# alenzhao/Mitty

Measured on AMD Instinct MI355X. Metric: paired 2x150bp reads/sec at 30x WGS, 1/2/4/8 MI355X; qname POS/CIGAR bit-exact, higher is better.
Workload: dtype int64+u8

## Files before the change

### include/mitty_hip.h

```cpp
#ifndef MITTY_HIP_H
#define MITTY_HIP_H

#include <stdint.h>

#ifdef __cplusplus
extern "C" {
#endif

typedef struct mh_ctx mh_ctx;

enum {
  MH_OK = 0,
  MH_E_ARG = -1,
  MH_E_HIP = -2,
  MH_E_OOM = -3,
  MH_E_CAPACITY = -4,
  MH_E_COMPLEX_VARIANT = -5,
  MH_E_SEED = -6,
  MH_E_STATE = -7,
  MH_E_NO_DEVICE = -8
};

enum { MH_RNG_MITTY = 0, MH_RNG_PHILOX = 1 };

// ... 111 lines not shown
int32_t mh_bam_export(mh_ctx *ctx, int64_t r0, int64_t r1, uint8_t *recs, int64_t *roff, uint64_t *keys,
                      int32_t *info);
int32_t mh_bam_import(mh_ctx *ctx, const uint8_t *recs, const int64_t *roff, const uint64_t *keys, const int32_t *info,
                      int64_t n);
int32_t mh_bam_write_gpu(mh_ctx *ctx, const char *bam_path, const char *header_text, int64_t header_len,
                         const char *bai_path, int64_t *out_records, int64_t *out_bytes, int64_t *out_file_bytes);
int32_t mh_bam_partition(mh_ctx *ctx, const uint64_t *splitters, int32_t n_dest, uint64_t tie_base, int64_t *seg_off,
                         int64_t *seg_n, int64_t *seg_bytes);
int32_t mh_bam_partition_fetch(mh_ctx *ctx, void *out, int64_t cap);
int32_t mh_bam_import_tie(mh_ctx *ctx, const uint8_t *recs, const int64_t *roff, const uint64_t *keys,
                          const int32_t *info, const uint64_t *ties, int64_t n);
int32_t mh_bam_sorted_head(mh_ctx *ctx, int64_t len, uint8_t *out);
int32_t mh_bam_write_part(mh_ctx *ctx, const char *path, const char *header_text, int64_t header_len, int64_t skip,
                          const uint8_t *tail, int64_t tail_len, int32_t eof, int64_t *out_blocks, int64_t *out_data_pos,
                          int64_t *out_bytes, int64_t *boff, int64_t boff_cap);
int32_t mh_bam_bai_runs(mh_ctx *ctx, int64_t *n_runs, int64_t *runs, int64_t runs_cap, int64_t *n_win, int64_t *win,
                        int64_t win_cap, int64_t *ref_nwin);

typedef struct mh_bamfile mh_bamfile;
int32_t mh_bamfile_open(const char *path, int32_t threads, mh_bamfile **out);
const char *mh_bamfile_error(const mh_bamfile *f);
int32_t mh_bamfile_header(const mh_bamfile *f, const char **text, int64_t *text_len, int32_t *n_ref,
                          const char **names, const int64_t **lengths);
int32_t mh_bamfile_next(mh_bamfile *f, int64_t max_bytes, const uint8_t **recs, int64_t *len, const int64_t **roff,
                        int64_t *n);
int32_t mh_bamfile_close(mh_bamfile *f);

int32_t mh_score_begin(mh_ctx *ctx, int32_t n_refs, const char *names, int32_t max_d, int32_t max_v_len,
                       int32_t strict, const char *sample_prefix);
int32_t mh_score_add_records(mh_ctx *ctx, const uint8_t *recs, int64_t len, const int64_t *roff, int64_t n);
int32_t mh_score_add_store(mh_ctx *ctx);
int32_t mh_score_result(mh_ctx *ctx, uint64_t *mq_mat, uint64_t *derr_mat, int64_t *counts);
int32_t mh_score_reset(mh_ctx *ctx);

typedef struct mh_vcf mh_vcf;
int32_t mh_vcf_open(const char *path, const char *sample, mh_vcf **out);
const char *mh_vcf_error(const mh_vcf *v);
int32_t mh_vcf_close(mh_vcf *v);
int32_t mh_vcf_region(mh_vcf *v, const char *chrom, int64_t start0, int64_t end, int32_t *ploidy, int64_t *n_var,
                      int64_t *alt_bytes, int32_t cap);
int32_t mh_vcf_copy(mh_vcf *v, int32_t cpy, int64_t *pos, uint8_t *op, int64_t *oplen, int64_t *alt_off,
                    int64_t *alt_len, char *alt_pool);
int32_t mh_vcf_filter(const char *in_path, const char *sample, int32_t n_regions, const char *chroms,
                      const int64_t *start0, const int64_t *end, const char *out_path, int32_t bgzf, int32_t threads,
                      int64_t *n_written, int64_t *n_filtered, char *err, int32_t err_cap);

typedef struct mh_fasta mh_fasta;
int32_t mh_fasta_open(const char *path, const char *names, mh_fasta **out);
const char *mh_fasta_error(const mh_fasta *f);
int32_t mh_fasta_count(const mh_fasta *f, int32_t *n);
int32_t mh_fasta_contig(const mh_fasta *f, int32_t i, const char **name, const char **seq, int64_t *len);
int32_t mh_fasta_copy(const mh_fasta *f, int32_t i, char *dst);
int32_t mh_fasta_close(mh_fasta *f);

int32_t mh_bgzf_compress(const char *in, int64_t len, int32_t level, int32_t threads, char *out, int64_t cap,
                         int64_t *used);
int32_t mh_bgzf_eof(char *out28);
int32_t mh_bgzf_compress_device(mh_ctx *ctx, const void *d_in, int64_t len, void *d_out, int64_t cap,
                                int64_t *used);
int32_t mh_bgzf_compress_gpu(mh_ctx *ctx, const char *in, int64_t len, char *out, int64_t cap, int64_t *used);
int32_t mh_output_bgzf(mh_ctx *ctx, int32_t file, char *out, int64_t cap, int64_t *used);
int32_t mh_output_bgzf_range(mh_ctx *ctx, int32_t file, int64_t offset, int64_t len, char *out, int64_t cap,
                             int64_t *used);
int32_t mh_output_bgzf_pair(mh_ctx *ctx, int64_t offset, int64_t n1, int64_t n2, char *out1, int64_t cap1,
                            char *out2, int64_t cap2, int64_t *used1, int64_t *used2, int32_t *ticket);
int32_t mh_output_bgzf_wait(mh_ctx *ctx, int32_t ticket);

int32_t mh_corrupt_fastq(mh_ctx *ctx, const char *fq1, int64_t len1, const char *fq2, int64_t len2, int64_t t_base,
                         int64_t *used1, int64_t *used2, int64_t *templates);

int32_t mh_set_corruption(mh_ctx *ctx, int32_t enable, const double *cum_bq, int32_t max_bp, int32_t n_bq,
                          const double *phred_p, uint64_t seed);
int32_t mh_set_corruption_stream(mh_ctx *ctx, int32_t rng_mode, uint64_t seed, const uint32_t *key624, int32_t pos);
int32_t mh_get_corruption_stream(mh_ctx *ctx, uint32_t *key624, int32_t *pos, int64_t *words);

int32_t mh_stage_times(mh_ctx *ctx, const char **names, double *ms, int32_t cap, int32_t *n);
int32_t mh_enable_timing(mh_ctx *ctx, int32_t on);

int32_t mh_mt_window_at(uint32_t seed, uint64_t offset, uint32_t *out624);
int32_t mh_set_emit_mode(mh_ctx *ctx, int32_t mode);
#define MH_DEC_SEQUENTIAL 1
#define MH_DEC_FORCE_FIXUP 2
#define MH_DEC_FORCE_GEO 4
int32_t mh_set_decode_mode(mh_ctx *ctx, int32_t mode);
int32_t mh_fixup_count(mh_ctx *ctx, int64_t *n);

#ifdef __cplusplus
}
#endif
#endif
```

### mitty_amd/_native.py

```python
import ctypes
import os
import sys

import numpy as np

LIB_PATH = (os.environ.get('MH_LIB') or
            os.path.join(os.path.dirname(os.path.abspath(__file__)), '_lib', 'libmitty_hip.so'))

MH_OK, MH_E_ARG, MH_E_HIP, MH_E_OOM, MH_E_CAPACITY, MH_E_COMPLEX_VARIANT, MH_E_SEED, MH_E_STATE, MH_E_NO_DEVICE = \
  0, -1, -2, -3, -4, -5, -6, -7, -8
MH_RNG_MITTY, MH_RNG_PHILOX = 0, 1

EXPORTS = ['mh_version', 'mh_device_count', 'mh_create', 'mh_destroy', 'mh_last_error', 'mh_sync',
           'mh_selftest_scan_fault', 'mh_selftest_scan', 'mh_selftest_sort',
           'mh_read_model_params', 'mh_work_units', 'mh_upload_contig', 'mh_build_haplotype', 'mh_upload_variants', 'mh_build_haplotype_vset', 'mh_build_haplotypes_vset', 'mh_prefetch_haplotypes_vset', 'mh_release_variants', 'mh_get_nodes', 'mh_get_haplotype_aux',
           'mh_release_haplotype', 'mh_expand_variant', 'mh_sample_templates', 'mh_sample_templates_span', 'mh_set_templates',
           'mh_get_templates', 'mh_templates_export', 'mh_templates_import', 'mh_emit_reads', 'mh_emit_prepare', 'mh_emit_reads_async', 'mh_emit_collect', 'mh_output_size', 'mh_output_fetch', 'mh_output_reset', 'mh_host_alloc', 'mh_host_free', 'mh_device_cache_trim', 'mh_device_live_bytes',
           'mh_read_batch', 'mh_set_corruption', 'mh_set_corruption_stream', 'mh_get_corruption_stream', 'mh_stage_times', 'mh_enable_timing', 'mh_sample_units', 'mh_sample_units_async', 'mh_templates_count',
           'mh_use_templates', 'mh_release_templates', 'mh_mt_window_at', 'mh_fixup_count', 'mh_set_emit_mode', 'mh_set_decode_mode',
           'mh_emit_reads_range', 'mh_emit_measure', 'mh_count_kept', 'mh_bam_set_refs', 'mh_bam_add_fastq', 'mh_bam_add_output',
           'mh_bam_records', 'mh_bam_set_capacity', 'mh_bam_set_spill_dir', 'mh_bam_spilled', 'mh_bam_export', 'mh_bam_import', 'mh_bam_sort', 'mh_bam_write', 'mh_bam_write_gpu', 'mh_bam_reset', 'mh_bam_partition', 'mh_bam_partition_fetch', 'mh_bam_import_tie', 'mh_bam_sorted_head', 'mh_bam_write_part', 'mh_bam_bai_runs', 'mh_corrupt_fastq', 'mh_bgzf_compress', 'mh_bgzf_eof', 'mh_bgzf_compress_device', 'mh_bgzf_compress_gpu', 'mh_output_bgzf',
           'mh_output_bgzf_range', 'mh_output_bgzf_pair', 'mh_output_bgzf_wait', 'mh_output_fetch_async',
           'mh_output_fetch_wait',
           'mh_vcf_open', 'mh_vcf_error', 'mh_vcf_close', 'mh_vcf_region', 'mh_vcf_copy', 'mh_vcf_filter',
           'mh_bamfile_open', 'mh_bamfile_error', 'mh_bamfile_header', 'mh_bamfile_next', 'mh_bamfile_close',
           'mh_score_begin', 'mh_score_add_records', 'mh_score_add_store', 'mh_score_result', 'mh_score_reset',
           'mh_fasta_open', 'mh_fasta_error', 'mh_fasta_count', 'mh_fasta_contig', 'mh_fasta_copy', 'mh_fasta_close']


class NativeError(RuntimeError):
  pass


class NativeUnavailable(NativeError):
  pass


_lib = None

c_i32, c_i64, c_u64, c_dbl, c_vp = ctypes.c_int32, ctypes.c_int64, ctypes.c_uint64, ctypes.c_double, ctypes.c_void_p
P_i64 = ctypes.POINTER(c_i64)


def _sig(L, name, args, res=c_i32):
  f = getattr(L, name)
  f.argtypes = args
  f.restype = res


def lib():
  global _lib
  if _lib is not None:
    return _lib
  if not os.path.exists(LIB_PATH):
    raise NativeUnavailable('libmitty_hip.so not built ({}); run __graft_entry__.build() or make -C '
                            'mitty_amd/csrc'.format(LIB_PATH))
  if 'torch' not in sys.modules and int(os.environ.get('WORLD_SIZE', '1')) > 1:
    import torch
  L = ctypes.CDLL(LIB_PATH)
  _sig(L, 'mh_version', [])
  _sig(L, 'mh_device_count', [ctypes.POINTER(c_i32)])
  _sig(L, 'mh_create', [c_i32, ctypes.POINTER(c_vp)])
  _sig(L, 'mh_destroy', [c_vp])
  _sig(L, 'mh_last_error', [c_vp], ctypes.c_char_p)
  _sig(L, 'mh_sync', [c_vp])
  _sig(L, 'mh_selftest_scan_fault', [c_vp])
  _sig(L, 'mh_selftest_scan', [c_vp, c_i32, c_i32, c_vp, c_i64, c_i32, c_vp, c_vp, c_vp, c_vp])
  _sig(L, 'mh_selftest_sort', [c_vp, c_vp, c_i64, c_i32, c_vp, c_vp])
  _sig(L, 'mh_read_model_params', [c_i64, c_dbl, ctypes.POINTER(c_dbl), P_i64])
  _sig(L, 'mh_work_units', [c_u64, c_vp, c_i64, c_i64, c_vp, c_vp, c_vp, P_i64])
  _sig(L, 'mh_upload_contig', [c_vp, c_i32, c_vp, c_i64])
  _sig(L, 'mh_upload_variants', [c_vp, c_i32, c_vp, c_vp, c_vp, c_vp, c_vp, c_vp, c_i64, c_i64])
  _sig(L, 'mh_build_haplotype_vset', [c_vp, c_i32, c_i32, c_i64, c_i32, c_vp, c_vp, c_vp])
  _sig(L, 'mh_release_variants', [c_vp, c_i32])
  _sig(L, 'mh_build_haplotype', [c_vp, c_i32, c_i32, c_i64, c_vp, c_vp, c_vp, c_vp, c_vp, c_vp, c_i64, c_i64,
                                 P_i64, P_i64, P_i64])
  _sig(L, 'mh_get_nodes', [c_vp, c_i32, c_vp, c_vp, c_vp, c_vp, c_vp, c_i64, P_i64])
  _sig(L, 'mh_get_haplotype_aux', [c_vp, c_i32, c_vp, c_i64, P_i64, c_vp, c_vp, c_i64, P_i64, c_vp, c_i64, P_i64])
  _sig(L, 'mh_release_haplotype', [c_vp, c_i32])
  _sig(L, 'mh_bgzf_compress_device', [c_vp, c_vp, c_i64, c_vp, c_i64, P_i64])
  _sig(L, 'mh_bgzf_compress_gpu', [c_vp, c_vp, c_i64, c_vp, c_i64, P_i64])
  _sig(L, 'mh_output_bgzf', [c_vp, c_i32, c_vp, c_i64, P_i64])
  _sig(L, 'mh_output_bgzf_range', [c_vp, c_i32, c_i64, c_i64, c_vp, c_i64, P_i64])
  _sig(L, 'mh_output_bgzf_pair', [c_vp, c_i64, c_i64, c_i64, c_vp, c_i64, c_vp, c_i64, P_i64, P_i64,
                                  ctypes.POINTER(c_i32)])
  _sig(L, 'mh_output_bgzf_wait', [c_vp, c_i32])
  _sig(L, 'mh_output_fetch_async', [c_vp, c_i64, c_vp, c_i64, c_i64, c_vp, c_i64, ctypes.POINTER(c_i32)])
  _sig(L, 'mh_output_fetch_wait', [c_vp, c_i32])
  _sig(L, 'mh_expand_variant', [c_i64, c_i64, c_i64, c_i64, c_i32, c_i64, P_i64, ctypes.POINTER(c_i32), P_i64, P_i64])
  _sig(L, 'mh_sample_templates', [c_vp, c_i32, c_dbl, c_i32, c_vp, c_i32, c_u64, c_i32, P_i64])
  _sig(L, 'mh_sample_templates_span', [c_vp, c_i64, c_i64, c_dbl, c_i32, c_vp, c_i32, c_u64, c_i32, P_i64])
  _sig(L, 'mh_set_templates', [c_vp, c_vp, c_vp, c_vp, c_i64, c_i32])
  _sig(L, 'mh_get_templates', [c_vp, c_vp, c_vp, c_vp, c_i64, P_i64])
  _sig(L, 'mh_emit_reads', [c_vp, c_i32, ctypes.c_char_p, ctypes.c_char_p, c_i64, c_i32, c_u64, P_i64, P_i64, P_i64])
  _sig(L, 'mh_emit_prepare', [c_vp, c_i32, ctypes.c_char_p, ctypes.c_char_p, c_i64, c_i32, c_u64, P_i64, P_i64, P_i64])
  _sig(L, 'mh_emit_reads_async', [c_vp, c_i32, ctypes.c_char_p, ctypes.c_char_p, c_i64, c_i32, c_u64])
  _sig(L, 'mh_emit_collect', [c_vp, c_vp, c_i64, P_i64])
  _sig(L, 'mh_build_haplotypes_vset', [c_vp, c_i32, c_vp, c_vp, c_vp, c_vp, c_vp, c_vp, c_vp])
  _sig(L, 'mh_prefetch_haplotypes_vset', [c_vp, c_i32, c_vp, c_vp, c_vp, c_vp, c_i32, c_vp, c_vp, c_dbl])
  _sig(L, 'mh_emit_reads_range', [c_vp, c_i32, ctypes.c_char_p, ctypes.c_char_p, c_i64, c_i32, c_u64, c_i64, c_i64,
                                   c_i64, P_i64, P_i64, P_i64])
  _sig(L, 'mh_count_kept', [c_vp, c_i32, c_i64, c_i64, P_i64])
  _sig(L, 'mh_emit_measure', [c_vp, c_i32, ctypes.c_char_p, ctypes.c_char_p, c_i64, c_i32, c_u64, c_i64, c_i64, c_i64,
                              P_i64, P_i64, P_i64])
  _sig(L, 'mh_bam_set_refs', [c_vp, c_i32, ctypes.c_char_p, c_vp])
  _sig(L, 'mh_bam_add_fastq', [c_vp, c_vp, c_i64, c_vp, c_i64, c_i64, P_i64, P_i64, P_i64])
  _sig(L, 'mh_bam_add_output', [c_vp, c_i64, P_i64])
  _sig(L, 'mh_bam_records', [c_vp, P_i64, P_i64])
  _sig(L, 'mh_bam_set_capacity', [c_vp, c_i64])
  _sig(L, 'mh_bam_spilled', [c_vp, P_i64, P_i64])
  _sig(L, 'mh_bam_export', [c_vp, c_i64, c_i64, c_vp, c_vp, c_vp, c_vp])
  _sig(L, 'mh_bam_import', [c_vp, c_vp, c_vp, c_vp, c_vp, c_i64])
  _sig(L, 'mh_bam_partition', [c_vp, c_vp, c_i32, ctypes.c_uint64, c_vp, c_vp, c_vp])
  _sig(L, 'mh_bam_set_spill_dir', [c_vp, ctypes.c_char_p])
  _sig(L, 'mh_bam_partition_fetch', [c_vp, c_vp, c_i64])
  _sig(L, 'mh_bam_import_tie', [c_vp, c_vp, c_vp, c_vp, c_vp, c_vp, c_i64])
  _sig(L, 'mh_bam_sorted_head', [c_vp, c_i64, c_vp])
  _sig(L, 'mh_bam_write_part', [c_vp, ctypes.c_char_p, ctypes.c_char_p, c_i64, c_i64, c_vp, c_i64, c_i32, P_i64,
                                P_i64, P_i64, c_vp, c_i64])
  _sig(L, 'mh_bam_bai_runs', [c_vp, P_i64, c_vp, c_i64, P_i64, c_vp, c_i64, c_vp])
  _sig(L, 'mh_bam_write', [c_vp, ctypes.c_char_p, ctypes.c_char_p, c_i64, c_i32, c_i32, ctypes.c_char_p, P_i64,
                           P_i64])
  _sig(L, 'mh_bam_write_gpu', [c_vp, ctypes.c_char_p, ctypes.c_char_p, c_i64, ctypes.c_char_p, P_i64, P_i64, P_i64])
  _sig(L, 'mh_bam_reset', [c_vp])
  _sig(L, 'mh_bam_sort', [c_vp])
  _sig(L, 'mh_corrupt_fastq', [c_vp, c_vp, c_i64, c_vp, c_i64, c_i64, P_i64, P_i64, P_i64])
  _sig(L, 'mh_bgzf_compress', [c_vp, c_i64, c_i32, c_i32, c_vp, c_i64, P_i64])
  _sig(L, 'mh_bgzf_eof', [c_vp])
  _sig(L, 'mh_vcf_open', [ctypes.c_char_p, ctypes.c_char_p, ctypes.POINTER(c_vp)])
  _sig(L, 'mh_vcf_error', [c_vp], ctypes.c_char_p)
  _sig(L, 'mh_vcf_close', [c_vp])
  _sig(L, 'mh_vcf_region', [c_vp, ctypes.c_char_p, c_i64, c_i64, ctypes.POINTER(c_i32), c_vp, c_vp, c_i32])
  _sig(L, 'mh_vcf_copy', [c_vp, c_i32, c_vp, c_vp, c_vp, c_vp, c_vp, c_vp])
  _sig(L, 'mh_vcf_filter', [ctypes.c_char_p, ctypes.c_char_p, c_i32, c_vp, c_vp, c_vp, ctypes.c_char_p, c_i32, c_i32,
                            P_i64, P_i64, ctypes.c_char_p, c_i32])
  _sig(L, 'mh_bamfile_open', [ctypes.c_char_p, c_i32, ctypes.POINTER(c_vp)])
  _sig(L, 'mh_bamfile_error', [c_vp], ctypes.c_char_p)
  _sig(L, 'mh_bamfile_header', [c_vp, ctypes.POINTER(c_vp), P_i64, ctypes.POINTER(c_i32), ctypes.POINTER(c_vp),
                                ctypes.POINTER(c_vp)])
  _sig(L, 'mh_bamfile_next', [c_vp, c_i64, ctypes.POINTER(c_vp), P_i64, ctypes.POINTER(c_vp), P_i64])
  _sig(L, 'mh_bamfile_close', [c_vp])
  _sig(L, 'mh_score_begin', [c_vp, c_i32, ctypes.c_char_p, c_i32, c_i32, c_i32, ctypes.c_char_p])
  _sig(L, 'mh_score_add_records', [c_vp, c_vp, c_i64, c_vp, c_i64])
  _sig(L, 'mh_score_add_store', [c_vp])
  _sig(L, 'mh_score_result', [c_vp, c_vp, c_vp, c_vp])
  _sig(L, 'mh_score_reset', [c_vp])
  _sig(L, 'mh_fasta_open', [ctypes.c_char_p, c_vp, ctypes.POINTER(c_vp)])
  _sig(L, 'mh_fasta_error', [c_vp], ctypes.c_char_p)
  _sig(L, 'mh_fasta_count', [c_vp, ctypes.POINTER(c_i32)])
  _sig(L, 'mh_fasta_contig', [c_vp, c_i32, ctypes.POINTER(ctypes.c_char_p), ctypes.POINTER(c_vp), P_i64])
  _sig(L, 'mh_fasta_copy', [c_vp, c_i32, c_vp])
  _sig(L, 'mh_fasta_close', [c_vp])
  _sig(L, 'mh_output_size', [c_vp, P_i64, P_i64])
  _sig(L, 'mh_output_fetch', [c_vp, c_i64, c_vp, c_i64, c_i64, c_vp, c_i64])
  _sig(L, 'mh_output_reset', [c_vp])
  _sig(L, 'mh_host_alloc', [c_i64, ctypes.POINTER(c_vp)])
  _sig(L, 'mh_host_free', [c_vp])
  _sig(L, 'mh_device_cache_trim', [ctypes.POINTER(c_i64)])
  _sig(L, 'mh_device_live_bytes', [ctypes.POINTER(c_i64), ctypes.POINTER(c_i64), c_i32])
  _sig(L, 'mh_read_batch', [c_vp, c_i32, c_vp, c_vp, c_i64, c_vp, c_vp, c_vp,
                            c_vp, c_i64, c_vp, P_i64, c_vp, c_i64, c_vp, P_i64, c_vp, c_i64, c_vp, P_i64])
  _sig(L, 'mh_set_corruption', [c_vp, c_i32, c_vp, c_i32, c_i32, c_vp, c_u64])
  _sig(L, 'mh_templates_export', [c_vp, c_i32, c_i32, c_vp, c_vp, c_vp, c_i64, P_i64])
  _sig(L, 'mh_templates_import', [c_vp, c_i32, c_i32, c_vp, c_vp, c_vp, c_i64, c_i32])
  _sig(L, 'mh_set_corruption_stream', [c_vp, c_i32, c_u64, c_vp, c_i32])
  _sig(L, 'mh_get_corruption_stream', [c_vp, c_vp, ctypes.POINTER(c_i32), P_i64])
  _sig(L, 'mh_stage_times', [c_vp, ctypes.POINTER(ctypes.c_char_p), ctypes.POINTER(c_dbl), c_i32,
                             ctypes.POINTER(c_i32)])
  _sig(L, 'mh_enable_timing', [c_vp, c_i32])
  _sig(L, 'mh_sample_units', [c_vp, c_i32, c_vp, c_vp, c_vp, c_dbl, c_i32, c_vp, c_i32, c_i32, c_vp])
  _sig(L, 'mh_sample_units_async', [c_vp, c_i32, c_vp, c_vp, c_vp, c_dbl, c_i32, c_vp, c_i32, c_i32])
  _sig(L, 'mh_templates_count', [c_vp, c_i32, c_vp])
  _sig(L, 'mh_use_templates', [c_vp, c_i32])
  _sig(L, 'mh_release_templates', [c_vp, c_i32])
  _sig(L, 'mh_mt_window_at', [ctypes.c_uint32, c_u64, c_vp])
  _sig(L, 'mh_fixup_count', [c_vp, P_i64])
  _sig(L, 'mh_set_emit_mode', [c_vp, c_i32])
  _sig(L, 'mh_set_decode_mode', [c_vp, c_i32])
  _lib = L
  return L


def mt_window_at(seed, offset):
  out = np.empty(624, np.uint32)
  rc = lib().mh_mt_window_at(int(seed), int(offset), _ptr(out))
  if rc:
    _raise(rc, 'mh_mt_window_at failed')
  return out


def bgzf_compress(data, level=6, threads=8):
  n = len(data)
  src = np.frombuffer(data, np.uint8) if n else np.zeros(1, np.uint8)
  cap = n + (n // 0xff00 + 1) * 64 + 64
  out = np.empty(cap, np.uint8)
  used = c_i64()
  rc = lib().mh_bgzf_compress(_ptr(src), n, int(level), int(threads), _ptr(out), cap, ctypes.byref(used))
  if rc == MH_E_CAPACITY:
    out = np.empty(used.value, np.uint8)
    rc = lib().mh_bgzf_compress(_ptr(src), n, int(level), int(threads), _ptr(out), used.value, ctypes.byref(used))
  if rc:
    _raise(rc, 'mh_bgzf_compress failed')
  return out[:used.value].tobytes()


class VcfFile:

  def __init__(self, path, sample):
    L = lib()
    self._L = L
    self._h = c_vp()
    rc = L.mh_vcf_open(path.encode(), sample.encode(), ctypes.byref(self._h))
    if rc:
      msg = L.mh_vcf_error(self._h).decode() if self._h else 'mh_vcf_open failed'
      self.close()
      _raise(rc, msg)

  def close(self):
    if getattr(self, '_h', None):
      self._L.mh_vcf_close(self._h)
      self._h = None

  def __del__(self):
    try:
      self.close()
    except Exception:
      pass

  def region(self, chrom, start0, end):
    pl = c_i32()
    nv = np.zeros(64, np.int64)
    ab = np.zeros(64, np.int64)
    rc = self._L.mh_vcf_region(self._h, chrom.encode(), int(start0), int(end), ctypes.byref(pl), _ptr(nv), _ptr(ab),
                               64)
    if rc:
      _raise(rc, self._L.mh_vcf_error(self._h).decode())
    copies = []
    for c in range(pl.value):
      n, nb = int(nv[c]), int(ab[c])
      pos, oplen, aoff, alen = (np.empty(n, np.int64) for _ in range(4))
      op = np.empty(n, np.uint8)
      pool = np.empty(max(nb, 1), np.uint8)
      rc = self._L.mh_vcf_copy(self._h, c, _ptr(pos), _ptr(op), _ptr(oplen), _ptr(aoff), _ptr(alen), _ptr(pool))
      if rc:
        _raise(rc, self._L.mh_vcf_error(self._h).decode())
      copies.append({'pos': pos, 'op': op, 'oplen': oplen, 'alt_off': aoff, 'alt_len': alen,
                     'alt_pool': pool[:nb].tobytes()})
    return pl.value, copies


class BamFile:

  def __init__(self, path, threads=2):
    L = lib()
    self._L = L
    self._h = c_vp()
    rc = L.mh_bamfile_open(path.encode(), int(threads), ctypes.byref(self._h))
    if rc:
      msg = L.mh_bamfile_error(self._h).decode(errors='replace') if self._h else 'mh_bamfile_open failed'
# ... 269 lines not shown
    self._chk(self._L.mh_release_variants(self._h, int(vset)))

  def get_nodes(self, slot, n_nodes, with_hap=True):
    ps, pr, ol = (np.empty(max(n_nodes, 1), np.int64) for _ in range(3))
    op = np.empty(max(n_nodes, 1), np.uint8)
    hl = c_i64()
    self._chk(self._L.mh_get_nodes(self._h, slot, None, None, None, None, None, 0, ctypes.byref(hl)))
    hap = np.empty(max(hl.value, 1), np.uint8) if with_hap else None
    self._chk(self._L.mh_get_nodes(self._h, slot, _ptr(ps), _ptr(pr), _ptr(op), _ptr(ol), _ptr(hap),
                                   hl.value if with_hap else 0, ctypes.byref(hl)))
    return ps[:n_nodes], pr[:n_nodes], op[:n_nodes], ol[:n_nodes], (hap[:hl.value].tobytes() if with_hap else None)

  def get_haplotype_aux(self, slot):
    hl, nr, nb = c_i64(), c_i64(), c_i64()
    self._chk(self._L.mh_get_haplotype_aux(self._h, slot, None, 0, ctypes.byref(hl), None, None, 0, ctypes.byref(nr),
                                           None, 0, ctypes.byref(nb)))
    rc = np.empty(max(hl.value, 1), np.uint8)
    rs, re_ = np.empty(max(nr.value, 1), np.int64), np.empty(max(nr.value, 1), np.int64)
    bkt = np.empty(nb.value + 1, np.int32)
    self._chk(self._L.mh_get_haplotype_aux(self._h, slot, _ptr(rc), hl.value, ctypes.byref(hl), _ptr(rs), _ptr(re_),
                                           nr.value, ctypes.byref(nr), _ptr(bkt), nb.value + 1, ctypes.byref(nb)))
    return rc[:hl.value].tobytes(), rs[:nr.value], re_[:nr.value], bkt

  def release_haplotype(self, slot):
    self._chk(self._L.mh_release_haplotype(self._h, slot))

  def sample_templates(self, slot, p, rlen, cum_tlen, seed, rng_mode=MH_RNG_MITTY):
    ct = np.ascontiguousarray(cum_tlen, dtype=np.float64)
    n = c_i64()
    self._chk(self._L.mh_sample_templates(self._h, slot, float(p), int(rlen), _ptr(ct), len(ct), int(seed),
                                          int(rng_mode), ctypes.byref(n)))
    return n.value

  def sample_templates_span(self, p_min, p_max, p, rlen, cum_tlen, seed, rng_mode=MH_RNG_MITTY):
    if not (0 <= int(seed) <= 0xffffffff):
      raise ValueError('Seed value {} is out of range 0 - {}'.format(seed, 0xffffffff))
    ct = np.ascontiguousarray(cum_tlen, dtype=np.float64)
    n = c_i64()
    self._chk(self._L.mh_sample_templates_span(self._h, int(p_min), int(p_max), float(p), int(rlen), _ptr(ct),
                                               len(ct), int(seed), int(rng_mode), ctypes.byref(n)))
    return n.value

  def sample_units(self, tpl_ids, slots, seeds, p, rlen, cum_tlen, rng_mode=MH_RNG_MITTY):
    ids = np.ascontiguousarray(tpl_ids, dtype=np.int32)
    sl = np.ascontiguousarray(slots, dtype=np.int32)
    sd = np.ascontiguousarray(seeds, dtype=np.uint64)
    ct = np.ascontiguousarray(cum_tlen, dtype=np.float64)
    out = np.zeros(max(len(ids), 1), dtype=np.int64)
    self._chk(self._L.mh_sample_units(self._h, len(ids), _ptr(ids), _ptr(sl), _ptr(sd), float(p), int(rlen),
                                      _ptr(ct), len(ct), int(rng_mode), _ptr(out)))
    return out[:len(ids)]

  def sample_units_async(self, tpl_ids, slots, seeds, p, rlen, cum_tlen, rng_mode=MH_RNG_MITTY):
    ids = np.ascontiguousarray(tpl_ids, dtype=np.int32)
    sl = np.ascontiguousarray(slots, dtype=np.int32)
    sd = np.ascontiguousarray(seeds, dtype=np.uint64)
    ct = np.ascontiguousarray(cum_tlen, dtype=np.float64)
    self._chk(self._L.mh_sample_units_async(self._h, len(ids), _ptr(ids), _ptr(sl), _ptr(sd), float(p), int(rlen),
                                            _ptr(ct), len(ct), int(rng_mode)))
    return len(ids)

  def template_count(self, tpl_id):
    n = c_i64()
    self._chk(self._L.mh_templates_count(self._h, int(tpl_id), ctypes.byref(n)))
    return n.value

  def use_templates(self, tpl_id):
    self._chk(self._L.mh_use_templates(self._h, int(tpl_id)))

  def release_templates(self, tpl_id):
    self._chk(self._L.mh_release_templates(self._h, int(tpl_id)))

  def set_emit_mode(self, mode):
    self._chk(self._L.mh_set_emit_mode(self._h, int(mode)))

  def set_decode_mode(self, mode):
    self._chk(self._L.mh_set_decode_mode(self._h, int(mode)))

  def fixup_count(self):
    n = c_i64()
    self._chk(self._L.mh_fixup_count(self._h, ctypes.byref(n)))
    return n.value

  def set_templates(self, fo0, pos0, pos1, rlen):
    fo0 = np.ascontiguousarray(fo0, dtype=np.int8)
    pos0 = np.ascontiguousarray(pos0, dtype=np.int64)
    pos1 = np.ascontiguousarray(pos1, dtype=np.int64)
    self._chk(self._L.mh_set_templates(self._h, _ptr(fo0), _ptr(pos0), _ptr(pos1), len(fo0), int(rlen)))

  def get_templates(self):
    n = c_i64()
    self._L.mh_get_templates(self._h, None, None, None, 0, ctypes.byref(n))
    m = n.value
    fo0, p0, p1 = np.empty(max(m, 1), np.int8), np.empty(max(m, 1), np.int64), np.empty(max(m, 1), np.int64)
    self._chk(self._L.mh_get_templates(self._h, _ptr(fo0), _ptr(p0), _ptr(p1), max(m, 1), ctypes.byref(n)))
    return fo0[:m], p0[:m], p1[:m]

  def emit_prepare(self, slot, serial_stub, chrom, cpy, write_fastq2=True, unit_key=0, wait=True):
    if not wait:
      self._chk(self._L.mh_emit_prepare(self._h, slot, serial_stub.encode(), chrom.encode(), int(cpy),
                                        1 if write_fastq2 else 0, int(unit_key), None, None, None))
      return None
    k, b1, b2 = c_i64(), c_i64(), c_i64()
    self._chk(self._L.mh_emit_prepare(self._h, slot, serial_stub.encode(), chrom.encode(), int(cpy),
                                      1 if write_fastq2 else 0, int(unit_key), ctypes.byref(k), ctypes.byref(b1),
                                      ctypes.byref(b2)))
    return k.value, b1.value, b2.value

  def emit_reads(self, slot, serial_stub, chrom, cpy, write_fastq2=True, unit_key=0, t_range=None, cnt_base=0):
    k, b1, b2 = c_i64(), c_i64(), c_i64()
    if t_range is None:
      self._chk(self._L.mh_emit_reads(self._h, slot, serial_stub.encode(), chrom.encode(), int(cpy),
                                      1 if write_fastq2 else 0, int(unit_key), ctypes.byref(k), ctypes.byref(b1),
                                      ctypes.byref(b2)))
    else:
      self._chk(self._L.mh_emit_reads_range(self._h, slot, serial_stub.encode(), chrom.encode(), int(cpy),
                                            1 if write_fastq2 else 0, int(unit_key), int(t_range[0]),
                                            int(t_range[1]), int(cnt_base), ctypes.byref(k), ctypes.byref(b1),
                                            ctypes.byref(b2)))
    return k.value, b1.value, b2.value

  def emit_async(self, slot, serial_stub, chrom, cpy, write_fastq2=True, unit_key=0):
    self._chk(self._L.mh_emit_reads_async(self._h, slot, serial_stub.encode(), chrom.encode(), int(cpy),
                                          1 if write_fastq2 else 0, int(unit_key)))

  def emit_collect(self):
    n = c_i64()
    self._chk(self._L.mh_emit_collect(self._h, None, 0, ctypes.byref(n)))
    out = np.zeros(3 * max(n.value, 1), np.int64)
    self._chk(self._L.mh_emit_collect(self._h, _ptr(out), n.value, ctypes.byref(n)))
    return [tuple(int(x) for x in out[3 * i:3 * i + 3]) for i in range(n.value)]

  def emit_measure(self, slot, serial_stub, chrom, cpy, write_fastq2=True, unit_key=0, t_range=None, cnt_base=0):
    k, b1, b2 = c_i64(), c_i64(), c_i64()
    t0, t1 = t_range if t_range is not None else (0, -1)
    self._chk(self._L.mh_emit_measure(self._h, slot, serial_stub.encode(), chrom.encode(), int(cpy),
                                      1 if write_fastq2 else 0, int(unit_key), int(t0), int(t1), int(cnt_base),
                                      ctypes.byref(k), ctypes.byref(b1), ctypes.byref(b2)))
    return k.value, b1.value, (b2.value if write_fastq2 else 0)

  def bgzf_range(self, f, off, n, pin):
    if n <= 0:
      return b''
    cap = n + (n // 0xff00 + 2) * 40 + 64
    pin.reserve(cap)
    used = c_i64()
    self._chk(self._L.mh_output_bgzf_range(self._h, int(f), int(off), int(n), c_vp(pin.ptr), cap, ctypes.byref(used)))
    return bytes(pin.view(used.value))

  def count_kept(self, slot, t_begin, t_end):
    k = c_i64()
    self._chk(self._L.mh_count_kept(self._h, slot, int(t_begin), int(t_end), ctypes.byref(k)))
    return k.value

  def output_size(self):
    a, b = c_i64(), c_i64()
    self._chk(self._L.mh_output_size(self._h, ctypes.byref(a), ctypes.byref(b)))
    return a.value, b.value

  def fetch_output(self, off1=0, len1=None, off2=0, len2=None):
    u1, u2 = self.output_size()
    len1 = u1 - off1 if len1 is None else len1
    len2 = u2 - off2 if len2 is None else len2
    b1 = np.empty(max(len1, 1), np.uint8)
    b2 = np.empty(max(len2, 1), np.uint8)
    self._chk(self._L.mh_output_fetch(self._h, off1, _ptr(b1), len1, off2, _ptr(b2) if len2 > 0 else None, len2))
# ... 368 lines not shown
```

### mitty_amd/csrc/mh_api.hip

```cpp
#include <sys/mman.h>
#include <sys/syscall.h>
#include <unistd.h>

#include <algorithm>
#include <atomic>
#include <cctype>
#include <cstdio>
#include <unordered_map>
#include <chrono>
#include <cmath>
#include <condition_variable>
#include <cstring>
#include <map>
#include <mutex>
#include <thread>
#include <type_traits>

#include "mh_bgzf.h"
#include <vector>

#include "mh_corrupt.h"
#include "mh_internal.h"
#include "mh_scan.h"
#include "mh_sort.h"

namespace mh {
namespace jump {
void window_at(uint32_t seed, uint64_t J, uint32_t *out624);
}

static std::mutex g_err_mu;

int32_t hip_fail(mh_ctx *ctx, hipError_t e, const char *what, const char *file, int line) {
  if (ctx) {
    std::lock_guard<std::mutex> lk(g_err_mu);
    ctx->err = std::string("HIP error ") + hipGetErrorName(e) + " (" + hipGetErrorString(e) + ") in " + what + " at " +
               file + ":" + std::to_string(line);
  }
  return e == hipErrorOutOfMemory ? MH_E_OOM : MH_E_HIP;
}

int32_t arg_fail(mh_ctx *ctx, int32_t code, const std::string &msg) {
  if (ctx) {
    std::lock_guard<std::mutex> lk(g_err_mu);
    ctx->err = msg;
  }
  return code;
}

bool scan_fault_pending(const mh_ctx *ctx) {
  const uint32_t *h = scan_fault_host();
  return h && __atomic_load_n(h + (ctx ? ctx->fault_slot : 0), __ATOMIC_ACQUIRE) != 0;
}

void lane_thread_enter(mh_ctx *ctx) { scan_fault_slot = ctx->fault_slot; }

int32_t scan_fault_fail(mh_ctx *ctx) {
  const uint32_t v = scan_fault_take(ctx ? ctx->fault_slot : 0);
  if (v & 2u) return arg_fail(ctx, MH_E_STATE, "single-pass writer: a qname part exceeded the splice's bound (internal)");
  if (v & 4u) return arg_fail(ctx, MH_E_STATE, "single-pass writer: the arena reservation was too small (internal)");
  return arg_fail(ctx, MH_E_STATE, "a look-back scan's wait timed out (a broken ticket base or scratch): its offsets "
                                   "are wrong");
}

namespace {
struct CachedBlock {
  void *p;
  int dev;
};
std::mutex g_cache_mu;
std::multimap<size_t, CachedBlock> g_cache;
std::atomic<int64_t> g_live{0}, g_live_peak{0};

void live_add(int64_t d) {
  const int64_t v = g_live.fetch_add(d) + d;
  int64_t pk = g_live_peak.load();
  while (v > pk && !g_live_peak.compare_exchange_weak(pk, v)) {
  }
}

void cache_put(void *p, size_t cap) {
  live_add(-(int64_t)cap);
  int dev = 0;
  (void)hipGetDevice(&dev);
  (void)hipDeviceSynchronize();
  std::lock_guard<std::mutex> lk(g_cache_mu);
  g_cache.insert({cap, CachedBlock{p, dev}});
}

void *cache_take(size_t bytes, size_t *cap) {
  int dev = 0;
  (void)hipGetDevice(&dev);
  std::lock_guard<std::mutex> lk(g_cache_mu);
  for (auto it = g_cache.lower_bound(bytes); it != g_cache.end(); ++it)
    if (it->second.dev == dev) {
      void *p = it->second.p;
      *cap = it->first;
      g_cache.erase(it);
      return p;
    }
  return nullptr;
}

int64_t cache_trim(int dev) {
  std::vector<std::pair<void *, int>> out;
  int64_t freed = 0;
  {
    std::lock_guard<std::mutex> lk(g_cache_mu);
    for (auto it = g_cache.begin(); it != g_cache.end();)
      if (dev < 0 || it->second.dev == dev) {
        out.push_back({it->second.p, it->second.dev});
        freed += (int64_t)it->first;
        it = g_cache.erase(it);
      } else {
        ++it;
      }
  }
  int cur = 0;
  (void)hipGetDevice(&cur);
  for (auto &b : out) {
    if (b.second != cur) (void)hipSetDevice(b.second);
    (void)hipFree(b.first);
    if (b.second != cur) (void)hipSetDevice(cur);
  }
  return freed;
}

hipError_t dev_alloc(void **p, size_t bytes, size_t *cap) {
  if ((*p = cache_take(bytes, cap))) {
    live_add((int64_t)*cap);
    return hipSuccess;
  }
  hipError_t e = hipMalloc(p, bytes);
  if (e != hipSuccess) {
    (void)hipGetLastError();
    int dev = 0;
    (void)hipGetDevice(&dev);
    if (cache_trim(dev) > 0) e = hipMalloc(p, bytes);
  }
  if (e == hipSuccess) {
    *cap = bytes;
// ... 211 lines not shown
  __device__ void operator()(int64_t i, const T &in, const T &ex) const {
    incl[i] = in;
    excl[i] = ex;
  }
};

template <typename T>
int32_t selftest_scan_run(mh_ctx *ctx, int32_t kind, const int64_t *in, int64_t n, int32_t repeat, int64_t *incl,
                          int64_t *excl, int64_t *total, int64_t *info) {
  hipStream_t st = ctx->stream;
  MH_TRY(ensure(ctx, ctx->scan_partials,
                kind == 2 ? scan_lb_scratch_bytes<T>(n) : sizeof(T) * (size_t)scan_partials_count(n) + 64));
  DevBuf b;
  const size_t ab = (sizeof(T) * (size_t)n + 255) & ~(size_t)255;
  MH_TRY(ensure(ctx, b, 3 * ab + 256));
  T *d_in = (T *)b.p, *d_incl = (T *)((char *)b.p + ab), *d_excl = (T *)((char *)b.p + 2 * ab);
  T *d_tot = (T *)((char *)b.p + 3 * ab);
  const int32_t rc = [&]() -> int32_t {
    if (n) HIPCHK(ctx, hipMemcpyAsync(d_in, in, sizeof(T) * (size_t)n, hipMemcpyHostToDevice, st));
    HIPCHK(ctx, hipMemsetAsync(d_incl, 0xff, 2 * ab + 256, st));
    const LoadArr<T> load{d_in};
    const StoreBoth<T> store{d_incl, d_excl};
    for (int32_t r = 0; r < repeat; r++) {
      if (kind == 0)
        HIPCHK(ctx, device_scan<T>(st, n, load, store, OpSum{}, T{}, (T *)ctx->scan_partials.p, d_tot));
      else if (kind == 1) {
        if constexpr (std::is_same<T, int64_t>::value)
          HIPCHK(ctx, device_scan<T>(st, n, load, store, OpMax{}, INT64_MIN, (T *)ctx->scan_partials.p, d_tot));
      } else if (kind == 2)
        HIPCHK(ctx, device_scan_sum<T>(st, n, load, store, ctx->scan_partials.p, d_tot));
      else
        HIPCHK(ctx, device_reduce<T>(st, n, load, OpSum{}, T{}, (T *)ctx->scan_partials.p, d_tot));
    }
    if (kind == 2) {
      std::lock_guard<std::mutex> lk(lb_mu());
      auto it = lb_states().find(ctx->scan_partials.p);
      if (it == lb_states().end()) return arg_fail(ctx, MH_E_HIP, "the look-back scratch has no state after a launch");
      info[0] = (int64_t)it->second.epoch;
      info[1] = (int64_t)(it->second.ticket - (uint32_t)scan_partials_count(n));
    }
    if (n && kind != 3) {
      HIPCHK(ctx, hipMemcpyAsync(incl, d_incl, sizeof(T) * (size_t)n, hipMemcpyDeviceToHost, st));
      HIPCHK(ctx, hipMemcpyAsync(excl, d_excl, sizeof(T) * (size_t)n, hipMemcpyDeviceToHost, st));
    }
    HIPCHK(ctx, hipMemcpyAsync(total, d_tot, sizeof(T), hipMemcpyDeviceToHost, st));
    SYNCCHK(ctx, hipStreamSynchronize(st));
    return MH_OK;
  }();
  release(b);
  return rc;
}
static_assert(LB_TILE == SCAN_TILE, "selftest_scan_run counts look-back tiles with scan_partials_count");
}

extern "C" {

int32_t mh_version(void) { return 1; }

int32_t mh_device_count(int32_t *out) {
  int n = 0;
  hipError_t e = hipGetDeviceCount(&n);
  if (e != hipSuccess) {
    (void)hipGetLastError();
    n = 0;
  }
  *out = n;
  return MH_OK;
}

int32_t mh_create(int32_t device, mh_ctx **out) {
  if (!out) return MH_E_ARG;
  *out = nullptr;
  int n = 0;
  if (hipGetDeviceCount(&n) != hipSuccess || n == 0) {
    (void)hipGetLastError();
    return MH_E_NO_DEVICE;
  }
  if (device < 0 || device >= n) return MH_E_ARG;
  mh_ctx *ctx = new mh_ctx();
  ctx->device = device;
  {
    static std::atomic<int> next{0};
    ctx->fault_slot = 1 + next++ % (SCAN_FAULT_SLOTS - 1);
    (void)scan_fault_take(ctx->fault_slot);
  }
  int prio_lo = 0, prio_hi = 0;
  (void)hipSetDevice(device);
  (void)hipDeviceGetStreamPriorityRange(&prio_lo, &prio_hi);
  if (hipSetDevice(device) != hipSuccess ||
      hipStreamCreateWithPriority(&ctx->stream, hipStreamNonBlocking, prio_hi) != hipSuccess ||
      hipStreamCreateWithPriority(&ctx->stream2, hipStreamNonBlocking, prio_hi) != hipSuccess ||
      hipEventCreateWithFlags(&ctx->ev_fork, hipEventDisableTiming) != hipSuccess ||
      hipEventCreateWithFlags(&ctx->ev_join, hipEventDisableTiming) != hipSuccess ||
      hipStreamCreateWithPriority(&ctx->wstream, hipStreamNonBlocking, prio_lo) != hipSuccess ||
      hipEventCreateWithFlags(&ctx->ev_ready, hipEventDisableTiming) != hipSuccess ||
      hipEventCreateWithFlags(&ctx->ev_writer, hipEventDisableTiming) != hipSuccess ||
      [&] {
        for (auto &e : ctx->eset)
          if (hipEventCreateWithFlags(&e.done, hipEventDisableTiming) != hipSuccess ||
              hipEventCreateWithFlags(&e.rb, hipEventDisableTiming) != hipSuccess ||
              hipHostMalloc((void **)&e.h_stat, 64 + 8192, hipHostMallocDefault) != hipSuccess)
            return true;
        return false;
      }()) {
    delete ctx;
    return MH_E_HIP;
  }
  hipDeviceProp_t prop;
  if (hipGetDeviceProperties(&prop, device) == hipSuccess) ctx->max_cu = prop.multiProcessorCount;
  *out = ctx;
  return MH_OK;
}

int32_t mh_destroy(mh_ctx *ctx) {
  if (!ctx) return MH_OK;
  if (ctx->pf_thread.joinable()) ctx->pf_thread.join();
  (void)hipSetDevice(ctx->device);
  (void)hipStreamSynchronize(ctx->wstream);
  (void)hipStreamSynchronize(ctx->stream);
  if (ctx->stream2) (void)hipStreamSynchronize(ctx->stream2);
  if (ctx->pstream) (void)hipStreamSynchronize(ctx->pstream);
  for (auto x : ctx->xstream)
    if (x) (void)hipStreamSynchronize(x);
  for (auto &kv : ctx->contigs) release(kv.second.seq);
  for (auto &kv : ctx->haps) release_hap(kv.second);
  for (auto &h : ctx->hap_spare) release_hap(h);
  for (auto &kv : ctx->vsets) release_vars(kv.second);
  for (auto &kv : ctx->tsets) {
    release(kv.second.fo0); release(kv.second.pos0); release(kv.second.pos1); release(kv.second.n0);
    if (kv.second.used) (void)hipEventDestroy(kv.second.used);
  }
  release(ctx->jump_polys); release(ctx->perm_tmp); release(ctx->nrun_tmp); release(ctx->dec_buf);
  for (auto &b : ctx->pb) release(b);
  release(ctx->pb_tmp);
  release(ctx->gz_slots); release(ctx->gz_tok); release(ctx->gz_info); release(ctx->gz_off); release(ctx->gz_scan); release(ctx->gz_out);
  release(ctx->gz_in);
  for (auto &b : ctx->s) release(b);
  for (auto &b : ctx->lane2) release(b);
  for (auto &l : ctx->xlane)
    for (auto &b : l) release(b);
  for (auto &b : ctx->xscan) release(b);
  release(ctx->scan_partials); release(ctx->scan_partials2); release(ctx->d_small);
  release(ctx->corrupt_cum); release(ctx->corrupt_phred);
  release(ctx->out1); release(ctx->out2);
  release(ctx->cr_rows);
  release(ctx->cr_codes);
  release(ctx->scan_partials_w);
  for (auto &b : ctx->sl2) release(b);
  for (auto &b : ctx->sl3) release(b);
  ctx->tail_state.reset();
  for (hipEvent_t e : ctx->ev_gz)
    if (e) (void)hipEventDestroy(e);
  for (hipEvent_t e : ctx->ev_fetch)
    if (e) (void)hipEventDestroy(e);
  if (ctx->h_small) (void)hipHostFree(ctx->h_small);
  if (ctx->h_small3) (void)hipHostFree(ctx->h_small3);
  if (ctx->h_units) (void)hipHostFree(ctx->h_units);
  for (uint8_t *p : ctx->h_bam_pin)
    if (p) (void)hipHostFree(p);
  for (auto &e : ctx->eset) {
    release(e.recs); release(e.off); release(e.tsum); release(e.tpre); release(e.stat); release(e.crrec);
    (void)hipEventDestroy(e.done);
    if (e.rb) (void)hipEventDestroy(e.rb);
    if (e.h_stat) (void)hipHostFree(e.h_stat);
  }
  (void)hipEventDestroy(ctx->ev_ready);
  (void)hipEventDestroy(ctx->ev_writer);
// ... 20 lines not shown
  CTX_GUARD(ctx);
  MH_TRY(lazy_resolve(ctx));
  SYNCCHK(ctx, hipStreamSynchronize(ctx->stream));
  return MH_OK;
}

namespace {
struct LoadOne {
  __device__ int64_t operator()(int64_t) const { return 1; }
};
struct StoreCheck {
  int32_t *bad;
  __device__ void operator()(int64_t i, int64_t, int64_t ex) const {
    if (ex != i) atomicOr(bad, 1);
  }
};
}

int32_t mh_selftest_sort(mh_ctx *ctx, const uint32_t *keys, int64_t n, int32_t end_bit, uint32_t *keys_out,
                         uint32_t *vals_out) {
  CTX_GUARD(ctx);
  if (n < 0 || (n > 0 && (!keys || !keys_out || !vals_out)) || end_bit < 0 || end_bit > 32)
    return arg_fail(ctx, MH_E_ARG, "bad sort arguments");
  hipStream_t st = ctx->stream;
  size_t tmp = 0;
  HIPCHK(ctx, lsd_sort_pairs_iota(nullptr, tmp, nullptr, nullptr, nullptr, n, (unsigned)end_bit, st));
  DevBuf b;
  const size_t kb = (4 * (size_t)n + 255) & ~(size_t)255;
  MH_TRY(ensure(ctx, b, 3 * kb + tmp + 256));
  uint32_t *dk = (uint32_t *)b.p, *ko = (uint32_t *)((char *)b.p + kb), *vo = (uint32_t *)((char *)b.p + 2 * kb);
  const int32_t rc = [&]() -> int32_t {
    if (n) HIPCHK(ctx, hipMemcpyAsync(dk, keys, 4 * (size_t)n, hipMemcpyHostToDevice, st));
    HIPCHK(ctx, lsd_sort_pairs_iota((char *)b.p + 3 * kb, tmp, dk, ko, vo, n, (unsigned)end_bit, st));
    if (n) {
      HIPCHK(ctx, hipMemcpyAsync(keys_out, ko, 4 * (size_t)n, hipMemcpyDeviceToHost, st));
      HIPCHK(ctx, hipMemcpyAsync(vals_out, vo, 4 * (size_t)n, hipMemcpyDeviceToHost, st));
    }
    SYNCCHK(ctx, hipStreamSynchronize(st));
    return MH_OK;
  }();
  release(b);
  return rc;
}

int32_t mh_selftest_scan(mh_ctx *ctx, int32_t kind, int32_t fields, const int64_t *in, int64_t n, int32_t repeat,
                         int64_t *incl, int64_t *excl, int64_t *total, int64_t *info) {
  CTX_GUARD(ctx);
  if (kind < 0 || kind > 3 || fields < 1 || fields > 3 || (kind == 1 && fields != 1) || n < 0 ||
      n > ((int64_t)1 << 27) || repeat < 1 || repeat > (1 << 20) || ((kind == 1 || kind == 3) && repeat != 1) ||
      !total || !info || (n > 0 && (!in || (kind != 3 && (!incl || !excl)))))
    return arg_fail(ctx, MH_E_ARG, "bad scan self-test arguments");
  if (kind == 2) {
    uint64_t sum[3] = {0, 0, 0};
    for (int64_t i = 0; i < n * fields; i++) {
      if (in[i] < 0) return arg_fail(ctx, MH_E_ARG, "look-back scan: a negative input");
      uint64_t &s = sum[i % fields];
      s += (uint64_t)in[i];
      if (s >= ((uint64_t)1 << 46)) return arg_fail(ctx, MH_E_ARG, "look-back scan: a field's total is 2^46 or more");
    }
  }
  info[0] = info[1] = 0;
  if (fields == 1) return selftest_scan_run<int64_t>(ctx, kind, in, n, repeat, incl, excl, total, info);
  if (fields == 2) return selftest_scan_run<Sc2>(ctx, kind, in, n, repeat, incl, excl, total, info);
  return selftest_scan_run<Sc3>(ctx, kind, in, n, repeat, incl, excl, total, info);
}

int32_t mh_selftest_scan_fault(mh_ctx *ctx) {
  CTX_GUARD(ctx);
  hipStream_t st = ctx->stream;
  const int64_t n = 2 * (int64_t)LB_TILE + 5;
  MH_TRY(ensure(ctx, ctx->scan_partials, scan_lb_scratch_bytes<int64_t>(n)));
  MH_TRY(ensure(ctx, ctx->scan_partials2, scan_lb_scratch_bytes<int64_t>(n)));
  MH_TRY(ensure(ctx, ctx->d_small, 8192 + 256));
  int64_t *tot = (int64_t *)((char *)ctx->d_small.p + 160);
  int32_t *bad = (int32_t *)((char *)ctx->d_small.p + 168);
  auto fault_once = [&](hipStream_t s, void *scratch) -> int32_t {
    HIPCHK(ctx, hipMemsetAsync(bad, 0, 4, s));
    HIPCHK(ctx, device_scan_sum<int64_t>(s, n, LoadOne{}, StoreCheck{bad}, scratch, tot, true));
    SYNCCHK(ctx, hipStreamSynchronize(s));
    return MH_OK;
  };
  int32_t rc_lane = MH_OK;
  std::thread t1([&]() {
    lane_thread_enter(ctx);
    if (hipSetDevice(ctx->device) != hipSuccess) {
      rc_lane = MH_E_HIP;
      return;
    }
    rc_lane = fault_once(ctx->stream2, ctx->scan_partials2.p);
  });
  t1.join();
  if (rc_lane != MH_E_STATE) return arg_fail(ctx, MH_E_HIP, "the timed-out scan of a lane thread was not reported");
  const int32_t rc = fault_once(st, ctx->scan_partials.p);
  if (rc != MH_E_STATE) return arg_fail(ctx, MH_E_HIP, "the timed-out scan was not reported");
  const std::string msg = ctx->err;
  HIPCHK(ctx, hipMemsetAsync(bad, 0, 4, st));
  HIPCHK(ctx, device_scan_sum<int64_t>(st, n, LoadOne{}, StoreCheck{bad}, ctx->scan_partials.p, tot));
  int32_t hb = 0;
  HIPCHK(ctx, hipMemcpyAsync(&hb, bad, 4, hipMemcpyDeviceToHost, st));
  SYNCCHK(ctx, hipStreamSynchronize(st));
  if (hb) return arg_fail(ctx, MH_E_HIP, "the scan after the fault is wrong");
  arg_fail(ctx, MH_E_STATE, msg);
  return MH_E_STATE;
}

int32_t mh_read_model_params(int64_t mean_rlen, double coverage, double *p_out, int64_t *passes_out) {
  if (!p_out || !passes_out || mean_rlen <= 0) return MH_E_ARG;
  double p = 1.0;
  int64_t passes = 1;
  while (p > 0.1) {
    passes *= 2;
    p = 0.5 * coverage / (double)(2 * mean_rlen * passes);
  }
  *p_out = p;
  *passes_out = passes;
  return MH_OK;
}

int32_t mh_work_units(uint64_t seed, const int32_t *ploidy, int64_t n_regions, int64_t passes, int32_t *out_region,
                      int32_t *out_cpy, uint32_t *out_seed, int64_t *out_n) {
  if (seed > 0xffffffffull) return MH_E_SEED;
  if (n_regions < 0 || passes < 0 || (n_regions && !ploidy)) return MH_E_ARG;
  HostMT s;
  s.seed((uint32_t)seed);
  uint32_t shuffle_seed = (uint32_t)s.interval(0xfffffffeull);
  int64_t n = 0;
  for (int64_t r = 0; r < n_regions; r++)
    for (int32_t c = 0; c < ploidy[r]; c++)
      for (int64_t k = 0; k < passes; k++) {
        out_region[n] = (int32_t)r;
        out_cpy[n] = c;
        out_seed[n] = (uint32_t)s.interval(0xfffffffeull);
        n++;
      }
  HostMT sh;
  sh.seed(shuffle_seed);
  for (int64_t i = n - 1; i >= 1; i--) {
    int64_t j = (int64_t)sh.interval((uint64_t)i);
    std::swap(out_region[i], out_region[j]);
    std::swap(out_cpy[i], out_cpy[j]);
    std::swap(out_seed[i], out_seed[j]);
  }
  *out_n = n;
  return MH_OK;
}

int32_t mh_upload_contig(mh_ctx *ctx, int32_t contig_id, const char *seq, int64_t len) {
  CTX_GUARD(ctx);
  if (len < 0 || (len > 0 && !seq)) return arg_fail(ctx, MH_E_ARG, "bad contig");
  Contig &c = ctx->contigs[contig_id];
  MH_TRY(ensure(ctx, c.seq, len + 16));
  if (len) HIPCHK(ctx, hipMemcpyAsync(c.seq.p, seq, len, hipMemcpyHostToDevice, ctx->stream));
  SYNCCHK(ctx, hipStreamSynchronize(ctx->stream));
  c.len = len;
  return MH_OK;
}

static int32_t hap_for_build(mh_ctx *ctx, int32_t slot, int64_t need, Hap **out, hipStream_t st = nullptr) {
  if (!ctx->haps.count(slot)) {
    int best = -1, big = -1;
    for (int i = 0; i < (int)ctx->hap_spare.size(); i++) {
      const Hap &s = ctx->hap_spare[i];
      if (s.used_set && hipEventQuery(s.used) != hipSuccess) continue;
      if (s.hap.cap >= (size_t)need && (best < 0 || s.hap.cap < ctx->hap_spare[best].hap.cap)) best = i;
      if (big < 0 || s.hap.cap > ctx->hap_spare[big].hap.cap) big = i;
    }
    if (best < 0) best = big;
// ... 13 lines not shown
  *out = &h;
  return MH_OK;
}

static int32_t build_from(mh_ctx *ctx, int32_t slot, int32_t contig_id, int64_t ref_start_pos, const VarSet &v,
                          int64_t *out_n_nodes, int64_t *out_p_min, int64_t *out_p_max) {
  auto it = ctx->contigs.find(contig_id);
  if (it == ctx->contigs.end()) return arg_fail(ctx, MH_E_STATE, "unknown contig id");
  Hap *hp = nullptr;
  MH_TRY(hap_for_build(ctx, slot, it->second.len + (it->second.len >> 6) + (1 << 20), &hp));
  Hap &h = *hp;
  MH_TRY(splice_build(ctx, h, it->second, ref_start_pos, v));
  if (out_n_nodes) *out_n_nodes = h.n_nodes;
  if (out_p_min) *out_p_min = h.p_min;
  if (out_p_max) *out_p_max = h.p_max;
  return MH_OK;
}

int32_t mh_build_haplotype(mh_ctx *ctx, int32_t slot, int32_t contig_id, int64_t ref_start_pos, const int64_t *v_pos,
                           const uint8_t *v_op, const int64_t *v_oplen, const int64_t *v_alt_off,
                           const int64_t *v_alt_len, const char *alt_pool, int64_t alt_pool_len, int64_t n_var,
                           int64_t *out_n_nodes, int64_t *out_p_min, int64_t *out_p_max) {
  CTX_GUARD_NOJOIN(ctx);
  if (!ctx->contigs.count(contig_id)) return arg_fail(ctx, MH_E_STATE, "unknown contig id");
  if (n_var < 0 || (n_var > 0 && (!v_pos || !v_op || !v_oplen || !v_alt_off || !v_alt_len)))
    return arg_fail(ctx, MH_E_ARG, "bad variant arrays");
  VarSet &v = ctx->vsets[-1];
  MH_TRY(var_upload(ctx, v, v_pos, v_op, v_oplen, v_alt_off, v_alt_len, alt_pool, alt_pool_len, n_var));
  return build_from(ctx, slot, contig_id, ref_start_pos, v, out_n_nodes, out_p_min, out_p_max);
}

int32_t mh_upload_variants(mh_ctx *ctx, int32_t vset, const int64_t *v_pos, const uint8_t *v_op,
                           const int64_t *v_oplen, const int64_t *v_alt_off, const int64_t *v_alt_len,
                           const char *alt_pool, int64_t alt_pool_len, int64_t n_var) {
  CTX_GUARD(ctx);
  if (vset < 0) return arg_fail(ctx, MH_E_ARG, "variant set ids are >= 0");
  if (n_var < 0 || (n_var > 0 && (!v_pos || !v_op || !v_oplen || !v_alt_off || !v_alt_len)))
    return arg_fail(ctx, MH_E_ARG, "bad variant arrays");
  const int32_t rc = var_upload(ctx, ctx->vsets[vset], v_pos, v_op, v_oplen, v_alt_off, v_alt_len, alt_pool,
                                alt_pool_len, n_var);
  if (rc != MH_OK) {
    release_vars(ctx->vsets[vset]);
    ctx->vsets.erase(vset);
  }
  return rc;
}

int32_t mh_build_haplotype_vset(mh_ctx *ctx, int32_t slot, int32_t contig_id, int64_t ref_start_pos, int32_t vset,
                                int64_t *out_n_nodes, int64_t *out_p_min, int64_t *out_p_max) {
  CTX_GUARD_NOJOIN(ctx);
  auto it = ctx->vsets.find(vset);
  if (vset < 0 || it == ctx->vsets.end()) return arg_fail(ctx, MH_E_STATE, "unknown variant set id");
  return build_from(ctx, slot, contig_id, ref_start_pos, it->second, out_n_nodes, out_p_min, out_p_max);
}

int32_t mh_build_haplotypes_vset(mh_ctx *ctx, int32_t n, const int32_t *slots, const int32_t *contig_ids,
                                 const int64_t *ref_starts, const int32_t *vsets, int64_t *out_n_nodes,
                                 int64_t *out_p_min, int64_t *out_p_max) {
  CTX_GUARD_NOJOIN(ctx);
  if (n < 0 || (n > 0 && (!slots || !contig_ids || !ref_starts || !vsets))) return arg_fail(ctx, MH_E_ARG, "bad arguments");
  for (int32_t i = 0; i < n; i++) {
    if (!ctx->contigs.count(contig_ids[i])) return arg_fail(ctx, MH_E_STATE, "unknown contig id");
    if (vsets[i] < 0 || !ctx->vsets.count(vsets[i])) return arg_fail(ctx, MH_E_STATE, "unknown variant set id");
    for (int32_t j = 0; j < i; j++)
      if (slots[j] == slots[i]) return arg_fail(ctx, MH_E_ARG, "a slot appears twice");
  }
  if (!pinned_small(ctx)) return arg_fail(ctx, MH_E_OOM, "pinned host memory");
  for (int32_t i0 = 0; i0 < n; i0 += 2) {
    const int32_t k = n - i0 < 2 ? n - i0 : 2;
    Hap *hp[2] = {nullptr, nullptr};
    for (int32_t j = 0; j < k; j++) {
      const int64_t L = ctx->contigs[contig_ids[i0 + j]].len;
      MH_TRY(hap_for_build(ctx, slots[i0 + j], L + (L >> 6) + (1 << 20), &hp[j]));
    }
    if (k == 1) {
      MH_TRY(splice_build(ctx, *hp[0], ctx->contigs[contig_ids[i0]], ref_starts[i0], ctx->vsets[vsets[i0]]));
    } else {
      HIPCHK(ctx, hipEventRecord(ctx->ev_fork, ctx->stream));
      HIPCHK(ctx, hipStreamWaitEvent(ctx->stream2, ctx->ev_fork, 0));
      const Contig &c1 = ctx->contigs[contig_ids[i0 + 1]];
      const VarSet &v1 = ctx->vsets[vsets[i0 + 1]];
      int32_t rc1 = MH_OK;
      std::thread t1([&]() {
        lane_thread_enter(ctx);
        try {
          const hipError_t e = hipSetDevice(ctx->device);
          if (e != hipSuccess) {
            rc1 = hip_fail(ctx, e, "hipSetDevice (splice lane 1)", __FILE__, __LINE__);
            return;
          }
          rc1 = splice_build(ctx, *hp[1], c1, ref_starts[i0 + 1], v1, 1);
        } catch (const std::bad_alloc &) {
          rc1 = arg_fail(ctx, MH_E_OOM, "host memory (splice lane 1)");
        } catch (const std::exception &x) {
          rc1 = arg_fail(ctx, MH_E_STATE, std::string("splice lane 1: ") + x.what());
        } catch (...) {
          rc1 = arg_fail(ctx, MH_E_STATE, "splice lane 1: unknown exception");
        }
      });
      const int32_t rc0 = splice_build(ctx, *hp[0], ctx->contigs[contig_ids[i0]], ref_starts[i0],
                                       ctx->vsets[vsets[i0]]);
      t1.join();
      HIPCHK(ctx, hipEventRecord(ctx->ev_join, ctx->stream2));
      HIPCHK(ctx, hipStreamWaitEvent(ctx->stream, ctx->ev_join, 0));
      if (rc0 != MH_OK) return rc0;
      if (rc1 != MH_OK) return rc1;
    }
    for (int32_t j = 0; j < k; j++) {
      if (out_n_nodes) out_n_nodes[i0 + j] = hp[j]->n_nodes;
      if (out_p_min) out_p_min[i0 + j] = hp[j]->p_min;
      if (out_p_max) out_p_max[i0 + j] = hp[j]->p_max;
    }
  }
  return MH_OK;
}

int32_t mh_prefetch_haplotypes_vset(mh_ctx *ctx, int32_t n, const int32_t *slots, const int32_t *contig_ids,
                                    const int64_t *ref_starts, const int32_t *vsets, int32_t n_units,
                                    const int32_t *unit_slots, const uint64_t *unit_seeds, double p) {
  CTX_GUARD_EMIT(ctx);
  MH_TRY(join_prefetch(ctx));
  if (n < 0 || (n > 0 && (!slots || !contig_ids || !ref_starts || !vsets))) return arg_fail(ctx, MH_E_ARG, "bad arguments");
  if (n_units < 0 || (n_units > 0 && (!unit_slots || !unit_seeds || !(p > 0.0 && p <= 1.0))))
    return arg_fail(ctx, MH_E_ARG, "bad unit arguments");
  for (int32_t i = 0; i < n; i++) {
    if (!ctx->contigs.count(contig_ids[i])) return arg_fail(ctx, MH_E_STATE, "unknown contig id");
    if (vsets[i] < 0 || !ctx->vsets.count(vsets[i])) return arg_fail(ctx, MH_E_STATE, "unknown variant set id");
    if (ctx->haps.count(slots[i])) return arg_fail(ctx, MH_E_ARG, "prefetch into a live haplotype slot");
    for (int32_t j = 0; j < i; j++)
      if (slots[j] == slots[i]) return arg_fail(ctx, MH_E_ARG, "a slot appears twice");
  }
  if (n == 0 && n_units == 0) return MH_OK;
  if (!ctx->pstream) {
    int lo = 0, hi = 0;
    (void)hipDeviceGetStreamPriorityRange(&lo, &hi);
    HIPCHK(ctx, hipStreamCreateWithPriority(&ctx->pstream, hipStreamNonBlocking, hi));
    HIPCHK(ctx, hipEventCreateWithFlags(&ctx->ev_prefetch, hipEventDisableTiming));
  }
  if (!ctx->h_small3 && hipHostMalloc((void **)&ctx->h_small3, 4096, hipHostMallocDefault) != hipSuccess) {
    ctx->h_small3 = nullptr;
    return arg_fail(ctx, MH_E_OOM, "pinned host memory");
  }
  struct Job {
    Hap *h;
    const Contig *c;
    int64_t rs;
    const VarSet *v;
  };
  std::vector<Job> jobs;
  for (int32_t i = 0; i < n; i++) {
    const Contig &c = ctx->contigs[contig_ids[i]];
    Hap *hp = nullptr;
    MH_TRY(hap_for_build(ctx, slots[i], c.len + (c.len >> 6) + (1 << 20), &hp, ctx->pstream));
    hp->prefetched = true;
    jobs.push_back(Job{hp, &c, ref_starts[i], &ctx->vsets[vsets[i]]});
  }
  std::vector<const Hap *> uh(n_units);
  for (int32_t u = 0; u < n_units; u++) {
    auto it = ctx->haps.find(unit_slots[u]);
    if (it == ctx->haps.end() || (!it->second.valid && !it->second.prefetched))
      return arg_fail(ctx, MH_E_STATE, "empty haplotype slot");
    uh[u] = &it->second;
  }
  std::vector<uint64_t> useeds(unit_seeds, unit_seeds + n_units);
  ctx->pf_words.valid = false;
  ctx->prefetch_pending = true;
  ctx->pf_rc = MH_OK;
  ctx->pf_thread = std::thread([ctx, jobs, uh, useeds, p]() {
    int32_t rc = MH_OK;
    lane_thread_enter(ctx);
    try {
      const hipError_t e = hipSetDevice(ctx->device);
      if (e != hipSuccess) rc = hip_fail(ctx, e, "hipSetDevice (prefetch)", __FILE__, __LINE__);
      for (size_t k = 0; k < jobs.size() && rc == MH_OK; k++)
        rc = splice_build(ctx, *jobs[k].h, *jobs[k].c, jobs[k].rs, *jobs[k].v, 2);
      if (rc == MH_OK && !uh.empty()) {
        std::vector<int64_t> pmin(uh.size()), pmax(uh.size());
        for (size_t u = 0; u < uh.size(); u++) {
          pmin[u] = uh[u]->p_min;
          pmax[u] = uh[u]->p_max;
        }
        rc = prefetch_words(ctx, ctx->pstream, (int32_t)uh.size(), pmin.data(), pmax.data(), useeds.data(), p);
      }
      const hipError_t e2 = hipEventRecord(ctx->ev_prefetch, ctx->pstream);
      if (rc == MH_OK && e2 != hipSuccess) rc = hip_fail(ctx, e2, "hipEventRecord (prefetch)", __FILE__, __LINE__);
    } catch (const std::bad_alloc &) {
      rc = arg_fail(ctx, MH_E_OOM, "host memory (prefetch)");
    } catch (const std::exception &x) {
      rc = arg_fail(ctx, MH_E_STATE, std::string("prefetch: ") + x.what());
    } catch (...) {
      rc = arg_fail(ctx, MH_E_STATE, "prefetch: unknown exception");
    }
    ctx->pf_rc = rc;
  });
  return MH_OK;
}

int32_t mh_release_variants(mh_ctx *ctx, int32_t vset) {
  CTX_GUARD(ctx);
  auto it = ctx->vsets.find(vset);
  if (it == ctx->vsets.end()) return MH_OK;
  SYNCCHK(ctx, hipStreamSynchronize(ctx->stream));
  release_vars(it->second);
  ctx->vsets.erase(it);
  return MH_OK;
}

int32_t mh_get_nodes(mh_ctx *ctx, int32_t slot, int64_t *ps, int64_t *pr, uint8_t *op, int64_t *oplen, char *hap,
                     int64_t hap_cap, int64_t *hap_len) {
  CTX_GUARD(ctx);
  auto it = ctx->haps.find(slot);
  if (it == ctx->haps.end() || !it->second.valid) return arg_fail(ctx, MH_E_STATE, "empty haplotype slot");
  Hap &h = it->second;
  hipStream_t st = ctx->stream;
  size_t n = (size_t)h.n_nodes;
  if (ps) HIPCHK(ctx, hipMemcpyAsync(ps, h.ps.p, 8 * n, hipMemcpyDeviceToHost, st));
  if (pr) HIPCHK(ctx, hipMemcpyAsync(pr, h.pr.p, 8 * n, hipMemcpyDeviceToHost, st));
  if (op) HIPCHK(ctx, hipMemcpyAsync(op, h.op.p, n, hipMemcpyDeviceToHost, st));
  if (oplen) HIPCHK(ctx, hipMemcpyAsync(oplen, h.oplen.p, 8 * n, hipMemcpyDeviceToHost, st));
  if (hap_len) *hap_len = h.hap_len;
  if (hap) {
    if (hap_cap < h.hap_len) {
      SYNCCHK(ctx, hipStreamSynchronize(st));
      return arg_fail(ctx, MH_E_CAPACITY, "haplotype buffer too small");
    }
    if (h.hap_len) HIPCHK(ctx, hipMemcpyAsync(hap, h.hap.p, h.hap_len, hipMemcpyDeviceToHost, st));
  }
  SYNCCHK(ctx, hipStreamSynchronize(st));
  return MH_OK;
}

int32_t mh_get_haplotype_aux(mh_ctx *ctx, int32_t slot, char *rc, int64_t rc_cap, int64_t *hap_len, int64_t *run_start,
                             int64_t *run_end, int64_t run_cap, int64_t *n_runs, int32_t *bkt, int64_t bkt_cap,
                             int64_t *n_bkt) {
  CTX_GUARD(ctx);
  auto it = ctx->haps.find(slot);
  if (it == ctx->haps.end() || !it->second.valid) return arg_fail(ctx, MH_E_STATE, "empty haplotype slot");
  Hap &h = it->second;
  if (hap_len) *hap_len = h.hap_len;
  if (n_runs) *n_runs = h.n_runs;
  if (n_bkt) *n_bkt = h.n_bkt;
  if (rc && rc_cap < h.hap_len) return arg_fail(ctx, MH_E_CAPACITY, "reverse complement buffer too small");
  if ((run_start || run_end) && run_cap < h.n_runs) return arg_fail(ctx, MH_E_CAPACITY, "N-run buffers too small");
  if (bkt && bkt_cap < h.n_bkt + 1) return arg_fail(ctx, MH_E_CAPACITY, "bucket buffer too small");
  hipStream_t st = ctx->stream;
  const size_t nr = (size_t)h.n_runs;
  if (rc && h.hap_len) HIPCHK(ctx, hipMemcpyAsync(rc, h.rc.p, h.hap_len, hipMemcpyDeviceToHost, st));
  if (run_start && nr) HIPCHK(ctx, hipMemcpyAsync(run_start, h.nrun_s.p, 8 * nr, hipMemcpyDeviceToHost, st));
  if (run_end && nr) HIPCHK(ctx, hipMemcpyAsync(run_end, h.nrun_e.p, 8 * nr, hipMemcpyDeviceToHost, st));
  if (bkt) HIPCHK(ctx, hipMemcpyAsync(bkt, h.bkt.p, 4 * (size_t)(h.n_bkt + 1), hipMemcpyDeviceToHost, st));
  SYNCCHK(ctx, hipStreamSynchronize(st));
  return MH_OK;
}
// ... 534 lines not shown
  if (key624) std::copy(h.key, h.key + 624, key624);
  if (pos) *pos = h.pos;
  return MH_OK;
}

int32_t mh_host_alloc(int64_t bytes, void **out) {
  if (!out || bytes < 0) return MH_E_ARG;
  *out = nullptr;
  const size_t n = (size_t)(bytes > 0 ? bytes : 1);
  int dev = 0;
  const int node = hipGetDevice(&dev) == hipSuccess ? mh::gpu_numa_node(dev) : -1;
  if (node >= 0 && node < 1024) {
    void *p = mmap(nullptr, n, PROT_READ | PROT_WRITE, MAP_PRIVATE | MAP_ANONYMOUS, -1, 0);
    if (p != MAP_FAILED) {
      unsigned long mask[1024 / (8 * sizeof(unsigned long))] = {0};
      mask[node / (8 * sizeof(unsigned long))] |= 1ul << (node % (8 * sizeof(unsigned long)));
      const long rc = syscall(SYS_mbind, p, n, 2 , mask, (unsigned long)1024, 0u);
      if (rc == 0 && hipHostRegister(p, n, hipHostRegisterDefault) == hipSuccess) {
        std::lock_guard<std::mutex> lk(mh::host_allocs_mu());
        mh::host_allocs()[p] = n;
        *out = p;
        return MH_OK;
      }
      (void)hipGetLastError();
      munmap(p, n);
    }
  }
  if (hipHostMalloc(out, n, hipHostMallocDefault) != hipSuccess) return MH_E_OOM;
  return MH_OK;
}

int32_t mh_device_cache_trim(int64_t *freed_bytes) {
  const int64_t f = mh::cache_trim(-1);
  if (freed_bytes) *freed_bytes = f;
  return MH_OK;
}

int32_t mh_device_live_bytes(int64_t *live, int64_t *peak, int32_t reset_peak) {
  if (live) *live = mh::g_live.load();
  if (peak) *peak = mh::g_live_peak.load();
  if (reset_peak) mh::g_live_peak.store(mh::g_live.load());
  return MH_OK;
}

int32_t mh_host_free(void *p) {
  if (!p) return MH_OK;
  size_t n = 0;
  {
    std::lock_guard<std::mutex> lk(mh::host_allocs_mu());
    auto it = mh::host_allocs().find(p);
    if (it != mh::host_allocs().end()) {
      n = it->second;
      mh::host_allocs().erase(it);
    }
  }
  if (n) {
    const hipError_t e = hipHostUnregister(p);
    munmap(p, n);
    return e == hipSuccess ? MH_OK : MH_E_HIP;
  }
  if (hipHostFree(p) != hipSuccess) return MH_E_HIP;
  return MH_OK;
}

int32_t mh_mt_window_at(uint32_t seed, uint64_t offset, uint32_t *out624) {
  if (!out624) return MH_E_ARG;
  try {
    mh::jump::window_at(seed, offset, out624);
  } catch (...) {
    return MH_E_ARG;
  }
  return MH_OK;
}

int32_t mh_set_emit_mode(mh_ctx *ctx, int32_t mode) {
  if (!ctx || mode < 0 || mode > 3) return MH_E_ARG;
  ctx->emit_lds_only = mode == 1;
  ctx->emit_two_pass = mode == 2;
  ctx->emit_single = mode == 3;
  return MH_OK;
}

int32_t mh_set_decode_mode(mh_ctx *ctx, int32_t mode) {
  if (!ctx || mode < 0 || mode > (MH_DEC_SEQUENTIAL | MH_DEC_FORCE_FIXUP | MH_DEC_FORCE_GEO)) return MH_E_ARG;
  ctx->decode_sequential = (mode & MH_DEC_SEQUENTIAL) != 0;
  ctx->force_fixup = (mode & MH_DEC_FORCE_FIXUP) != 0;
  ctx->force_geo = (mode & MH_DEC_FORCE_GEO) != 0;
  return MH_OK;
}

int32_t mh_fixup_count(mh_ctx *ctx, int64_t *n) {
  if (!ctx || !n) return MH_E_ARG;
  *n = ctx->fixups;
  return MH_OK;
}

int32_t mh_enable_timing(mh_ctx *ctx, int32_t on) {
  if (!ctx) return MH_E_ARG;
  (void)hipSetDevice(ctx->device);
  stages_collect(ctx);
  ctx->timing = on != 0;
  ctx->last_times.clear();
  return MH_OK;
}

int32_t mh_stage_times(mh_ctx *ctx, const char **names, double *ms, int32_t cap, int32_t *n) {
  if (!ctx || !n) return MH_E_ARG;
  (void)hipSetDevice(ctx->device);
  stages_collect(ctx);
  int32_t k = 0;
  for (auto &t : ctx->last_times) {
    if (k < cap) {
      if (names) names[k] = t.first;
      if (ms) ms[k] = t.second;
    }
    k++;
  }
  *n = k;
  if (names || ms) ctx->last_times.clear();
  return MH_OK;
}

int32_t mh_bam_set_refs(mh_ctx *ctx, int32_t n_refs, const char *names, const int64_t *lengths) {
  CTX_GUARD(ctx);
  if (n_refs < 0 || (n_refs > 0 && (!names || !lengths))) return arg_fail(ctx, MH_E_ARG, "bad reference list");
  return bam_set_refs(ctx, n_refs, names, lengths);
}

static int32_t stage_in(mh_ctx *ctx, DevBuf &b, const char *src, int64_t len) {
  MH_TRY(ensure(ctx, b, (size_t)len + 64));
  if (len) HIPCHK(ctx, hipMemcpyAsync(b.p, src, len, hipMemcpyHostToDevice, ctx->stream));
  HIPCHK(ctx, hipMemsetAsync((char *)b.p + len, 0, 64, ctx->stream));
  return MH_OK;
}

int32_t mh_bam_add_fastq(mh_ctx *ctx, const char *fq1, int64_t len1, const char *fq2, int64_t len2,
                         int64_t max_templates, int64_t *used1, int64_t *used2, int64_t *templates) {
  CTX_GUARD(ctx);
  if (!fq1 || len1 < 0 || (fq2 && len2 < 0) || !used1 || !used2 || !templates)
    return arg_fail(ctx, MH_E_ARG, "null argument");
  MH_TRY(stage_in(ctx, ctx->bam.in1, fq1, len1));
  if (fq2) MH_TRY(stage_in(ctx, ctx->bam.in2, fq2, len2));
  return bam_add(ctx, (const uint8_t *)ctx->bam.in1.p, len1, fq2 ? (const uint8_t *)ctx->bam.in2.p : nullptr,
                 fq2 ? len2 : 0, max_templates, used1, used2, templates);
}

int32_t mh_bam_add_output(mh_ctx *ctx, int64_t max_templates, int64_t *templates) {
  CTX_GUARD(ctx);
  MH_TRY(lazy_resolve(ctx));
  if (!templates) return arg_fail(ctx, MH_E_ARG, "null argument");
  int64_t u1 = 0, u2 = 0;
  const bool two = ctx->used2 > 0;
  const uint8_t *a1 = (const uint8_t *)ctx->out1.p, *a2 = two ? (const uint8_t *)ctx->out2.p : nullptr;
  if (ctx->bam.cap <= 0)
    return bam_add(ctx, a1, ctx->used1, a2, two ? ctx->used2 : 0, max_templates, &u1, &u2, templates, true);
  const int64_t per = std::max<int64_t>(1, ctx->bam.cap / 2048);
  int64_t o1 = 0, o2 = 0, tot = 0;
  int64_t win = per * 4096;
  while (max_templates < 0 || tot < max_templates) {
    const int64_t lim = max_templates < 0 ? per : std::min(per, max_templates - tot);
    const int64_t r1 = ctx->used1 - o1, r2 = two ? ctx->used2 - o2 : 0;
    const int64_t l1 = std::min(r1, win), l2 = std::min(r2, win);
    int64_t t = 0;
    MH_TRY(bam_add(ctx, a1 + o1, l1, two ? a2 + o2 : nullptr, l2, lim, &u1, &u2, &t, false));
    if (t == 0 && (l1 < r1 || l2 < r2)) {
      win *= 2;
      continue;
    }
    if (t == 0) break;
    o1 += u1;
    o2 += u2;
    tot += t;
  }
  *templates = tot;
  return MH_OK;
}
// ... 656 lines not shown
```

### mitty_amd/csrc/mh_internal.h

```cpp
#pragma once

#include <hip/hip_runtime.h>

#include <cstdint>
#include <functional>
#include <map>
#include <mutex>
#include <unordered_map>
#include <memory>
#include <string>
#include <thread>
#include <vector>

#include "../../include/mitty_hip.h"

namespace mh {

struct Status {
  int32_t code = MH_OK;
  std::string msg;
};

#define MH_TRY(expr)                        \
  do {                                      \
// ... 118 lines not shown
  int32_t pend = -1;
};

struct Contig {
  DevBuf seq;
  int64_t len = 0;
};

struct VarSet {
  DevBuf pos, op, oplen, aoff, alen, pool;
  int64_t n = 0, pool_len = 0;
};

struct BamStore {
  bool refs_set = false;
  std::vector<std::string> ref_names;
  std::vector<int64_t> ref_len;
  DevBuf names, name_off;
  DevBuf in1, in2;
  DevBuf nl1, nl2;
  DevBuf tpl;
  DevBuf roff, recs;
  DevBuf key, val, info;
  DevBuf key2, val2, sort_tmp, soff, srecs, sinfo;
  DevBuf bai_lin, bai_runs, bai_out;
  DevBuf tie, tie2, tval, tkey;
  DevBuf part_dest, part_dk, part_ord, part_soff, part_start, part_seg, part_split, part_tmp, send;
  bool use_tie = false;
  int64_t send_bytes = 0;
  int64_t n_rec = 0, bytes = 0;
  int32_t n_files = 0;
  bool sorted = false;
  bool direct = false;
  int64_t cap = 0;
  struct HostBlock {
    uint8_t *p;
    int64_t b0, b1;
    bool mapped = false;
  };
  std::vector<HostBlock> spill;
  int64_t spilled = 0;
  std::string spill_dir;
};

struct ScoreState {
  bool begun = false;
  int32_t max_d = 0, max_v = 0, strict = 0, n_refs = 0, plen = 0;
  int64_t n_mq = 0, n_dv = 0, n_all = 0;
  DevBuf acc, delta;
  DevBuf err;
  DevBuf names, name_off, prefix;
  DevBuf in[2];
  uint8_t *pin[2] = {nullptr, nullptr};
  size_t pin_cap[2] = {0, 0};
  hipEvent_t ev[2] = {nullptr, nullptr};
  bool ev_set[2] = {false, false};
  int cur = 0;
  int64_t base_rec = 0;
};

struct StageTime {
  const char *name;
  hipEvent_t a, b;
};

}

namespace mh {
struct EmitSet {
  DevBuf recs, off;
  DevBuf tsum, tpre;
  DevBuf crrec;
  DevBuf stat;
  int64_t *h_stat = nullptr;
  hipEvent_t rb = nullptr;
  hipEvent_t done = nullptr;
  bool busy = false;
  bool prepared = false;
};
}

struct mh_ctx {
  int fault_slot = 0;
  int device = 0;
  hipStream_t stream = nullptr;
  hipStream_t stream2 = nullptr;
  hipEvent_t ev_fork = nullptr, ev_join = nullptr;
  hipStream_t wstream = nullptr;
  std::shared_ptr<void> tail_state;
  int64_t *h_units = nullptr, *d_units = nullptr;
  hipEvent_t ev_ready = nullptr, ev_writer = nullptr;
  bool writer_pending = false;
  static constexpr int N_ESET = 16;
  mh::EmitSet eset[N_ESET];
  int64_t eset_max_m = 0;
  int eset_i = 0;
  hipStream_t stage_stream = nullptr;
  std::string err;
  int32_t max_cu = 256;

  std::map<int32_t, mh::Contig> contigs;
  std::map<int32_t, mh::Hap> haps;

  std::map<int32_t, mh::TplSet> tsets;
  int32_t cur_tpl = -1;

  mh::DevBuf jump_polys;
  int64_t jump_k = 0, jump_seg = 0;
  int64_t fixups = 0;
  std::map<int32_t, mh::VarSet> vsets;
  std::vector<mh::Hap> hap_spare;
  mh::DevBuf perm_tmp;
  mh::DevBuf pb[6];
  mh::DevBuf pb_tmp;
  mh::DevBuf gz_slots, gz_info, gz_off, gz_scan, gz_out, gz_in;
  mh::DevBuf gz_tok;
  hipEvent_t ev_gz[2] = {nullptr, nullptr};
  hipEvent_t ev_fetch[2] = {nullptr, nullptr};
  bool fetch_pending[2] = {false, false};
  int fetch_next = 0;
  bool gz_pending[2] = {false, false};
  int gz_half = 0;
  mh::DevBuf nrun_tmp;
  mh::DevBuf dec_buf;
  int64_t dec_passes = 0;

  mh::DevBuf s[16];
  mh::DevBuf scan_partials;
  mh::DevBuf lane2[8];
  mh::DevBuf scan_partials2;
  hipStream_t xstream[2] = {nullptr, nullptr};
  mh::DevBuf xlane[2][8];
  mh::DevBuf xscan[2];
  hipEvent_t ev_xjoin[2] = {nullptr, nullptr};
  mh::DevBuf sl2[8];
  hipStream_t pstream = nullptr;
  hipEvent_t ev_prefetch = nullptr;
  bool prefetch_pending = false;
  std::thread pf_thread;
  int32_t pf_rc = 0;
  mh::DevBuf sl3[8];
  int64_t *h_small3 = nullptr;
  mh::PrefetchedWords pf_words;
  mh::DevBuf pinned_small;
  mh::DevBuf d_small;

  bool corrupt_on = false;
  mh::DevBuf corrupt_cum, corrupt_phred;
  int32_t corrupt_max_bp = 0, corrupt_n_bq = 0;
  size_t corrupt_guide_off = 0;
  size_t corrupt_bk_off = 0, corrupt_T16_off = 0, corrupt_Fp16_off = 0;
  size_t corrupt_bkf_off = 0;
  uint64_t corrupt_seed = 0;
  int32_t cx_mode = 0;
  uint32_t cx_seed = 0;
  int64_t cx_pos = 0;
  uint32_t cx_key[624] = {0};
  int32_t cx_kpos = 624;
  mh::DevBuf cx_words, cx_bits, cx_start, cx_aux;

  bool emit_lds_only = false;
  bool decode_sequential = false;
  bool force_fixup = false;
  bool force_geo = false;

  mh::DevBuf out1, out2;
  int64_t used1 = 0, used2 = 0;
  static constexpr int LZ_SLOTS = 4096;
  int64_t *h_lazy = nullptr, *d_lazy = nullptr;
  mh::DevBuf d_cur;
  mh::DevBuf fused_lb;
  struct LazyUnit {
    int32_t slot;
    int64_t gen;
    int64_t known[3];
  };
  std::vector<LazyUnit> lazy;
  std::vector<int64_t> lazy_done;
  int64_t lazy_seq = 0;
  int64_t lazy_gen = 0;
  bool chain_open = false;
  int64_t used_ub1 = 0, used_ub2 = 0;
  int64_t batch_left = 0;
  bool emit_two_pass = false;
  bool emit_single = false;
  mh::DevBuf cr_rows, cr_codes;
  mh::DevBuf scan_partials_w;
  int64_t *h_small = nullptr;
  uint8_t *h_bam_pin[2] = {nullptr, nullptr};

  bool timing = false;
  std::vector<mh::StageTime> stages;
  std::vector<mh::StageTime> pending;
  std::vector<std::pair<const char *, double>> last_times;

  mh::BamStore bam;
  mh::ScoreState score;
};

namespace mh {

int32_t hip_fail(mh_ctx *ctx, hipError_t e, const char *what, const char *file, int line);
int32_t arg_fail(mh_ctx *ctx, int32_t code, const std::string &msg);

#define HIPCHK(ctx, call)                                                     \
  do {                                                                        \
    hipError_t _e = (call);                                                   \
    if (_e != hipSuccess) return ::mh::hip_fail((ctx), _e, #call, __FILE__, __LINE__); \
  } while (0)

int32_t scan_fault_fail(mh_ctx *ctx);
#define SYNCCHK(ctx, call)                                                    \
  do {                                                                        \
    HIPCHK(ctx, call);                                                        \
    if (::mh::scan_fault_pending(ctx)) return ::mh::scan_fault_fail(ctx);     \
  } while (0)
bool scan_fault_pending(const mh_ctx *ctx);

int32_t ensure(mh_ctx *ctx, DevBuf &b, size_t bytes);
int32_t ensure_keep(mh_ctx *ctx, DevBuf &b, size_t bytes, size_t keep, int32_t grow_shift = 1);
void release(DevBuf &b);
void release_hap(Hap &h);
int32_t join_writer(mh_ctx *ctx);
int32_t mark_used(mh_ctx *ctx, hipEvent_t &ev, bool &set);
int32_t wait_unused(mh_ctx *ctx, hipEvent_t ev, bool set, hipStream_t st = nullptr);
int32_t join_prefetch(mh_ctx *ctx);
int32_t prefetch_words(mh_ctx *ctx, hipStream_t st, int32_t n_units, const int64_t *p_min, const int64_t *p_max,
                       const uint64_t *seeds, double p);

void stage_begin(mh_ctx *ctx, const char *name);
void stage_end(mh_ctx *ctx);
void stages_collect(mh_ctx *ctx);

inline unsigned grid_for(int64_t n, int threads, int64_t cap = 1 << 20) {
  int64_t g = (n + threads - 1) / threads;
  if (g < 1) g = 1;
  if (g > cap) g = cap;
  return (unsigned)g;
}

int32_t var_upload(mh_ctx *ctx, VarSet &v, const int64_t *v_pos, const uint8_t *v_op, const int64_t *v_oplen,
                   const int64_t *v_alt_off, const int64_t *v_alt_len, const char *alt_pool, int64_t alt_pool_len,
                   int64_t n_var);
void release_vars(VarSet &v);
int32_t splice_build(mh_ctx *ctx, Hap &h, const Contig &c, int64_t ref_start_pos, const VarSet &v, int lane = 0);

int32_t sample_units(mh_ctx *ctx, int32_t n_units, const int32_t *tpl_ids, const int64_t *p_min, const int64_t *p_max,
                     const uint64_t *seeds, double p, int32_t rlen, const double *cum_tlen, int32_t n_tlen,
                     int32_t rng_mode, int64_t *out_n, const NodeIdx *nidx = nullptr);
int32_t sample_units_async(mh_ctx *ctx, int32_t n_units, const int32_t *tpl_ids, const int64_t *p_min,
                           const int64_t *p_max, const uint64_t *seeds, double p, int32_t rlen, const double *cum_tlen,
                           int32_t n_tlen, int32_t rng_mode, const NodeIdx *nidx = nullptr);
int32_t tpl_resolve(mh_ctx *ctx, TplSet &ts);
int32_t tpl_resolve_all(mh_ctx *ctx);

int32_t sync_writers(mh_ctx *ctx);
int32_t bgzf_device(mh_ctx *ctx, hipStream_t st, const uint8_t *d_in, int64_t n, uint8_t *d_out, int64_t cap,
                    int64_t *used, std::vector<int64_t> *boff = nullptr,
                    const std::function<void(int64_t, int64_t)> *on_piece = nullptr);
int64_t bgzf_device_bound(int64_t n);
int gpu_numa_node(int dev);
std::mutex &host_allocs_mu();
std::unordered_map<void *, size_t> &host_allocs();
int64_t *pinned_small(mh_ctx *ctx);
int32_t emit_reads(mh_ctx *ctx, const Hap &h, int32_t slot, const char *serial_stub, const char *chrom, int64_t cpy,
                   int32_t write_fastq2, uint64_t unit_key, int64_t t_begin, int64_t t_end, int64_t cnt_base,
                   bool prepare_only, int64_t *out_kept, int64_t *out_b1, int64_t *out_b2);
int32_t count_kept(mh_ctx *ctx, const Hap &h, int64_t t_begin, int64_t t_end, int64_t *out_kept);
int32_t emit_unit_async(mh_ctx *ctx, const Hap &h, const char *serial_stub, const char *chrom, int64_t cpy,
                        int32_t write_fastq2, uint64_t unit_key, bool *queued);
int32_t lazy_resolve(mh_ctx *ctx);

int32_t bam_set_refs(mh_ctx *ctx, int32_t n_refs, const char *names, const int64_t *lengths);
int32_t bam_add(mh_ctx *ctx, const uint8_t *d1, int64_t len1, const uint8_t *d2, int64_t len2, int64_t max_templates,
                int64_t *used1, int64_t *used2, int64_t *templates, bool sorted_direct = false);
int32_t bam_sort(mh_ctx *ctx, const void *pa = nullptr);
int32_t bam_undirect(mh_ctx *ctx);
int32_t bam_fetch_sorted(mh_ctx *ctx, uint8_t *recs, int64_t *soff, int32_t *info);
int32_t bam_spill(mh_ctx *ctx);
int32_t bam_export(mh_ctx *ctx, int64_t r0, int64_t r1, uint8_t *recs, int64_t *roff, uint64_t *key, int32_t *info);
int32_t bam_import(mh_ctx *ctx, const uint8_t *recs, const int64_t *roff, const uint64_t *key, const int32_t *info,
                   int64_t n, const uint64_t *tie = nullptr);
int32_t bam_partition(mh_ctx *ctx, const uint64_t *split, int32_t n_dest, uint64_t tie_base, int64_t *seg_off,
                      int64_t *seg_n, int64_t *seg_bytes);
int32_t bam_bai_raw(mh_ctx *ctx, std::vector<int64_t> &runs, std::vector<int64_t> &win, std::vector<uint32_t> &nwin,
                    std::vector<int64_t> &woff, bool *ok);
struct BamHostOrder {
  std::vector<uint32_t> val;
  std::vector<int64_t> roff, soff;
};
int32_t bam_host_order(mh_ctx *ctx, BamHostOrder &o);
void bam_assemble(const BamStore &B, const BamHostOrder &o, int64_t w0, int64_t w1, uint8_t *dst, int threads);
struct BaiPlan;
int32_t bam_bai_plan(mh_ctx *ctx, BaiPlan &plan, std::vector<int64_t> &offs, bool *ok);
// ... 38 lines not shown
```

### mitty_amd/csrc/mh_sample.hip

```cpp
#include <algorithm>
#include <cmath>
#include <cstdio>
#include <cstdlib>
#include <cstring>


#include "mh_device.h"
#include "mh_internal.h"
#include "mh_scan.h"
#include "mh_sort.h"


namespace mh {

namespace jump {
void jump_poly_words(uint64_t L, int64_t k, uint32_t *out624);
}

namespace {

constexpr uint32_t MT_UP = 0x80000000u, MT_LO = 0x7fffffffu, MT_A = 0x9908b0dfu;
constexpr int64_t SEG_WORDS_DEFAULT = 624 * 640;
static int64_t seg_words() { return SEG_WORDS_DEFAULT; }

// ... 75 lines not shown
      cb[CB_ZERO + i] = 0u;
    }
    lds_barrier();
    const int w = t < JW ? t : 0;
    uint32_t a0 = 0, a1 = 0, a2 = 0;
    int32_t G = 624;
    for (int pw = 0; pw < 624; pw++) {
      const int kb = pw * 32;
      while (G <= kb + 31 + 623) {
#pragma unroll
        for (int ph = 0; ph < 3; ph++) {
          if (t < (ph < 2 ? 227 : 170)) {
            const int i = G + 227 * ph + t;
            const uint32_t v = cb[(i - 227) & CB_MASK] ^ mt_mix(cb[(i - 624) & CB_MASK], cb[(i - 623) & CB_MASK]);
            cb[i & CB_MASK] = v;
            cb[(i & CB_MASK) + CB_WORDS] = v;
          }
          lds_barrier();
        }
        G += 624;
      }
      uint32_t m = __builtin_amdgcn_readfirstlane(gp[pw]);
      const int base = kb & CB_MASK;
      for (int nleft = __builtin_popcount(m); nleft > 0; nleft -= JB) {
        int off[JB];
#pragma unroll
        for (int u = 0; u < JB; u++) {
          off[u] = u < nleft ? base + __builtin_ctz(m) : CB_ZERO;
          m &= m - 1u;
        }
        uint32_t v0[JB], v1[JB], v2[JB];
#pragma unroll
        for (int u = 0; u < JB; u++) {
          const uint32_t *q = cb + off[u] + w;
          v0[u] = q[0];
          v1[u] = q[JW];
          v2[u] = q[2 * JW];
        }
#pragma unroll
        for (int u = 0; u < JB; u++) {
          a0 ^= v0[u];
          a1 ^= v1[u];
          a2 ^= v2[u];
        }
      }
    }
    lds_barrier();
    if (t < JW) {
      cb[t] = a0;
      cb[t + JW] = a1;
      cb[t + 2 * JW] = a2;
    }
    lds_barrier();
  }
  uint32_t *st0 = cb, *st1 = cb + 624;
  uint32_t *out = job.out + job.start;
  const int64_t cnt = job.count;
  for (int64_t base = 0; base < cnt; base += 624) {
    mt_twist_block(st0, st1, [&](int k, uint32_t w) {
      if (base + k < cnt) out[base + k] = w;
    });
    uint32_t *tmp = st0; st0 = st1; st1 = tmp;
  }
}

__device__ __forceinline__ uint32_t interval_mask(uint32_t m) {
  m |= m >> 1; m |= m >> 2; m |= m >> 4; m |= m >> 8; m |= m >> 16;
  return m;
}

struct DecJob {
  const uint32_t *words;
  int64_t n_words;
  int64_t n;
  uint32_t *j;
  int64_t *status;
};

constexpr int DC_THREADS = 256;
constexpr int DC_WAVES = DC_THREADS / 64;
constexpr int DC_PER = 4;
constexpr int DC_CHUNK = DC_THREADS * DC_PER;

__global__ void __launch_bounds__(DC_THREADS) k_shuffle_decode2(const DecJob *jobs) {
  __shared__ int32_t wsum[DC_WAVES];
  __shared__ int32_t s_tot;
  const DecJob job = jobs[blockIdx.x];
  const int t = threadIdx.x, lane = t & 63, wave = t >> 6;
  if (t == 0 && job.n > 0) job.j[0] = 0;
  int64_t i0 = job.n - 1;
  int64_t base = 0;
  float ratio = 0.75f;
  uint4 nxt = make_uint4(0, 0, 0, 0);
  if (DC_PER * t + 3 < job.n_words) nxt = *(const uint4 *)(job.words + DC_PER * t);
  while (i0 >= 1 && base < job.n_words) {
    uint32_t w[DC_PER] = {nxt.x, nxt.y, nxt.z, nxt.w};
    bool valid[DC_PER];
#pragma unroll
    for (int e = 0; e < DC_PER; e++) valid[e] = base + DC_PER * t + e < job.n_words;
    {
      const int64_t nb = base + DC_CHUNK + DC_PER * t;
      if (nb + 3 < job.n_words) nxt = *(const uint4 *)(job.words + nb);
    }
    int32_t A = (int32_t)(ratio * (float)(DC_PER * t));
    int32_t cnt = 0;
    uint32_t v[DC_PER];
    bool acc[DC_PER];
    bool converged = false;
    for (int it = 0; it < 24; it++) {
      cnt = 0;
#pragma unroll
      for (int e = 0; e < DC_PER; e++) {
        const int64_t i = i0 - A - cnt;
        v[e] = (i >= 1) ? (w[e] & interval_mask((uint32_t)i)) : 0u;
        acc[e] = valid[e] && i >= 1 && v[e] <= (uint32_t)i;
        cnt += acc[e];
      }
      int32_t incl = cnt;
#pragma unroll
      for (int d = 1; d < 64; d <<= 1) {
        int32_t o = __shfl_up(incl, d, 64);
        if (lane >= d) incl += o;
      }
      if (lane == 63) wsum[wave] = incl;
      __syncthreads();
      int32_t pre = 0, tot = 0;
#pragma unroll
      for (int q = 0; q < DC_WAVES; q++) {
        const int32_t s = wsum[q];
        pre += q < wave ? s : 0;
        tot += s;
      }
      const int32_t A2 = pre + incl - cnt;
      const int same = __syncthreads_and(A2 == A);
      A = A2;
      if (t == 0) s_tot = tot;
      if (same) {
        converged = true;
        break;
      }
    }
    if (!converged) {
      __syncthreads();
      if (t == 0) {
        int64_t ii = i0;
        for (int64_t k = 0; k < DC_CHUNK && base + k < job.n_words && ii >= 1; k++) {
          const uint32_t vv = job.words[base + k] & interval_mask((uint32_t)ii);
          if (vv <= (uint32_t)ii) { job.j[ii] = vv; ii--; }
        }
        s_tot = (int32_t)(i0 - ii);
      }
      __syncthreads();
    } else {
      int32_t a = 0;
#pragma unroll
      for (int e = 0; e < DC_PER; e++) {
        if (acc[e]) job.j[i0 - A - a] = v[e];
        a += acc[e];
      }
    }
    __syncthreads();
    const int32_t tot = s_tot;
    i0 -= tot;
    base += DC_CHUNK;
    ratio = (float)tot / (float)DC_CHUNK;
    __syncthreads();
  }
  if (t == 0) *job.status = i0 < 1 ? 0 : i0;
}
// ... 64 lines not shown
      int32_t o = __shfl_up(incl, d, 64);
      if (lane >= d) incl += o;
    }
    if (lane == 63) wsum[wave] = incl;
    __syncthreads();
    int32_t pre = 0, tot = 0;
#pragma unroll
    for (int q = 0; q < DC_WAVES; q++) {
      const int32_t s = wsum[q];
      pre += q < wave ? s : 0;
      tot += s;
    }
    const int32_t A2 = pre + incl - cnt;
    const int same = __syncthreads_and(A2 == A);
    A = A2;
    if (t == 0) s_tot = tot;
    if (same) {
      converged = true;
      break;
    }
  }
  if (!converged) {
    __syncthreads();
    if (t == 0) {
      int64_t ii = i0;
      int64_t lo = -DC_BIG, hi = DC_BIG;
      for (int64_t k = 0; k < job.size && base + k < job.n_words; k++) {
        if (ii < 1) { hi = 0; break; }
        const uint32_t m = interval_mask((uint32_t)ii);
        const uint32_t vv = job.words[base + k] & m;
        lo = max(lo, (int64_t)(m >> 1) + 1 - ii);
        hi = min(hi, (int64_t)m - ii);
        if (vv <= (uint32_t)ii) {
          lo = max(lo, (int64_t)vv - ii);
          if (WRITE) job.j[ii] = vv;
          ii--;
        } else {
          hi = min(hi, (int64_t)vv - ii - 1);
        }
      }
      count[c] = (int32_t)(i0 - ii);
      margin[2 * c] = (int32_t)lo;
      margin[2 * c + 1] = (int32_t)hi;
    }
    return;
  }
  int64_t lo = -DC_BIG, hi = DC_BIG;
  {
    int32_t a = 0;
#pragma unroll
    for (int e = 0; e < DC_PER; e++) {
      if (!valid[e]) continue;
      const int64_t i = i0 - A - a;
      if (i < 1) { hi = 0; continue; }
      const uint32_t m = interval_mask((uint32_t)i);
      lo = max(lo, (int64_t)(m >> 1) + 1 - i);
      hi = min(hi, (int64_t)m - i);
      if (acc[e]) lo = max(lo, (int64_t)v[e] - i); else hi = min(hi, (int64_t)v[e] - i - 1);
      if (WRITE && acc[e]) job.j[i] = v[e];
      a += acc[e];
    }
  }
  int32_t l32 = (int32_t)max(lo, (int64_t)-DC_BIG), h32 = (int32_t)min(hi, (int64_t)DC_BIG);
#pragma unroll
  for (int d = 32; d >= 1; d >>= 1) {
    l32 = max(l32, __shfl_xor(l32, d, 64));
    h32 = min(h32, __shfl_xor(h32, d, 64));
  }
  if (lane == 0) { wlo[wave] = l32; whi[wave] = h32; }
  __syncthreads();
  if (t == 0) {
    int32_t L = -DC_BIG, H = DC_BIG;
    for (int q = 0; q < DC_WAVES; q++) { L = max(L, wlo[q]); H = min(H, whi[q]); }
    count[c] = s_tot;
    margin[2 * c] = L;
    margin[2 * c + 1] = H;
  }
}

template <bool WRITE>
__global__ void __launch_bounds__(DC_THREADS) k_decode_chunks(const ChunkJob *jobs, const int32_t *todo,
                                                              const int32_t *n_todo, int32_t n_all,
                                                              const int64_t *start, int32_t *count,
                                                              int32_t *margin) {
  __shared__ int32_t wsum[DC_WAVES];
  __shared__ int32_t wlo[DC_WAVES], whi[DC_WAVES];
  __shared__ int32_t s_tot;
  const int32_t n = todo ? *n_todo : n_all;
  for (int32_t i = blockIdx.x; i < n; i += gridDim.x) {
    decode_chunk<WRITE>(jobs, todo ? todo[i] : i, start, count, margin, wsum, wlo, whi, s_tot);
    __syncthreads();
  }
}

constexpr int DR_THREADS = 256, DR_PER = 8, DR_TILE = DR_THREADS * DR_PER;
struct DecTile {
  int32_t unit, begin, end, first_tile;
};

__device__ __forceinline__ int64_t block_sum_dr(int64_t v, int64_t *wsum) {
  const int lane = threadIdx.x & 63, wave = threadIdx.x >> 6;
#pragma unroll
  for (int d = 32; d >= 1; d >>= 1) v += __shfl_xor(v, d, 64);
  if (lane == 0) wsum[wave] = v;
  __syncthreads();
  int64_t tot = 0;
#pragma unroll
  for (int q = 0; q < DR_THREADS / 64; q++) tot += wsum[q];
  return tot;
}

__global__ void __launch_bounds__(DR_THREADS) k_decode_resolve(const DecTile *tiles, const int64_t *n_draws,
                                                               const int32_t *count, const int32_t *margin,
                                                               int64_t *s0, int64_t *s1, int32_t *todo,
                                                               int32_t *n_todo, int32_t *n_next, int64_t *rem) {
  __shared__ int64_t wsum[DR_THREADS / 64];
  const int t = threadIdx.x, lane = t & 63, wave = t >> 6;
  const DecTile tl = tiles[blockIdx.x];
  if (blockIdx.x == 0 && t == 0) *n_next = 0;
  int64_t before = 0;
  for (int32_t k = tl.first_tile; k < (int32_t)blockIdx.x; k++) {
    const int32_t b = tiles[k].begin + t * DR_PER, e = tiles[k].end;
    int32_t cb[DR_PER];
#pragma unroll
    for (int q = 0; q < DR_PER; q++) cb[q] = b + q < e ? count[b + q] : 0;
#pragma unroll
    for (int q = 0; q < DR_PER; q++) before += cb[q];
  }
  const int64_t carry = n_draws[tl.unit] - 1 - block_sum_dr(before, wsum);
  __syncthreads();
  const int32_t c0 = tl.begin + t * DR_PER;
  int32_t cv[DR_PER];
  int64_t loc = 0;
#pragma unroll
  for (int k = 0; k < DR_PER; k++) {
    cv[k] = c0 + k < tl.end ? count[c0 + k] : 0;
    loc += cv[k];
  }
  int64_t incl = loc;
#pragma unroll
  for (int d = 1; d < 64; d <<= 1) {
    const int64_t o = __shfl_up(incl, d, 64);
    if (lane >= d) incl += o;
  }
  if (lane == 63) wsum[wave] = incl;
  __syncthreads();
  int64_t pre = 0;
#pragma unroll
  for (int q = 0; q < DR_THREADS / 64; q++) pre += q < wave ? wsum[q] : 0;
  int64_t s = carry - (pre + incl - loc);
  int64_t o0[DR_PER];
  int32_t mlo[DR_PER], mhi[DR_PER];
#pragma unroll
  for (int k = 0; k < DR_PER; k++) {
    const int32_t c = c0 + k < tl.end ? c0 + k : tl.begin;
    o0[k] = s0[c];
    mlo[k] = margin[2 * c];
    mhi[k] = margin[2 * c + 1];
  }
  uint32_t rq = 0;
#pragma unroll
  for (int k = 0; k < DR_PER; k++) {
    const int32_t c = c0 + k;
    if (c < tl.end) {
      const int64_t sv = s > 0 ? s : 0;
      s1[c] = sv;
      const int64_t d = sv - o0[k];
      if (d < mlo[k] || d > mhi[k]) {
        s0[c] = sv;
        rq |= 1u << k;
      }
    }
    s -= cv[k];
  }
  const int32_t nrq = __popc(rq);
  int32_t rincl = nrq;
#pragma unroll
  for (int d = 1; d < 64; d <<= 1) {
    const int32_t o = __shfl_up(rincl, d, 64);
    if (lane >= d) rincl += o;
  }
  const int32_t wtot = __shfl(rincl, 63, 64);
  if (wtot > 0) {
    int32_t q0 = 0;
    if (lane == 63) q0 = atomicAdd(n_todo, wtot);
    q0 = __shfl(q0, 63, 64) + rincl - nrq;
#pragma unroll
    for (int k = 0; k < DR_PER; k++)
      if (rq & (1u << k)) todo[q0++] = c0 + k;
  }
  if (t == DR_THREADS - 1 && (blockIdx.x + 1 == gridDim.x || tiles[blockIdx.x + 1].unit != tl.unit)) {
    const int64_t left = carry - (pre + incl);
    rem[tl.unit] = left < 1 ? 0 : left;
  }
}

struct TailJob {
  const uint32_t *words;
  int64_t n_words;
  int64_t base;
// ... 341 lines not shown
  mask |= mask >> 1; mask |= mask >> 2; mask |= mask >> 4; mask |= mask >> 8; mask |= mask >> 16; mask |= mask >> 32;
  if (max <= 0xffffffffull) {
    while ((v = (next() & mask)) > max) {}
  } else {
    while ((v = ((((uint64_t)next()) << 32 | next()) & mask)) > max) {}
  }
  return v;
}

namespace {

int32_t ensure_polys(mh_ctx *ctx, hipStream_t st, int64_t kmax, int64_t seg) {
  if (ctx->jump_k >= kmax + 1 && ctx->jump_seg == seg) return MH_OK;
  std::vector<uint32_t> polys((size_t)(kmax + 1) * 624);
  for (int64_t k = 0; k <= kmax; k++) jump::jump_poly_words((uint64_t)seg, k, polys.data() + k * 624);
  MH_TRY(ensure(ctx, ctx->jump_polys, 4 * polys.size()));
  HIPCHK(ctx, hipMemcpyAsync(ctx->jump_polys.p, polys.data(), 4 * polys.size(), hipMemcpyHostToDevice, st));
  SYNCCHK(ctx, hipStreamSynchronize(st));
  ctx->jump_k = kmax + 1;
  ctx->jump_seg = seg;
  return MH_OK;
}

__global__ void __launch_bounds__(256) k_mt_state(const uint32_t *key, int32_t pos, int64_t count, uint32_t *out) {
  __shared__ uint32_t st[2][624];
  for (int i = threadIdx.x; i < 624; i += 256) st[0][i] = key[i];
  lds_barrier();
  const int64_t lead = 624 - pos;
  for (int64_t i = threadIdx.x; i < lead && i < count; i += 256) out[i] = mt_temper(st[0][pos + i]);
  uint32_t *o = st[0], *nw = st[1];
  for (int64_t base = lead; base < count; base += 624) {
    mt_twist_block(o, nw, [&](int k, uint32_t w) {
      if (base + k < count) out[base + k] = w;
    });
    uint32_t *tmp = o; o = nw; nw = tmp;
  }
}

}

int32_t mt_stream_words(mh_ctx *ctx, hipStream_t st, uint32_t seed, int64_t first, int64_t count, DevBuf &out,
                        DevBuf &jobs_buf, int64_t *lead) {
  const int64_t SEG = seg_words();
  const int64_t k0 = first / SEG, k1 = (first + std::max<int64_t>(count, 1) - 1) / SEG;
  *lead = first - k0 * SEG;
  MH_TRY(ensure(ctx, out, 4 * (size_t)((k1 - k0 + 1) * SEG) + 64));
  std::vector<SegJob> jobs;
  for (int64_t k = k0; k <= k1; k++)
    jobs.push_back(SegJob{(uint32_t *)out.p, (k - k0) * SEG, std::min(SEG, first + count - k * SEG), seed, (int32_t)k});
  MH_TRY(ensure_polys(ctx, st, k1, SEG));
  MH_TRY(ensure(ctx, jobs_buf, sizeof(SegJob) * jobs.size() + 64));
  HIPCHK(ctx, hipMemcpyAsync(jobs_buf.p, jobs.data(), sizeof(SegJob) * jobs.size(), hipMemcpyHostToDevice, st));
  hipLaunchKernelGGL(k_mt_segments, dim3((unsigned)jobs.size()), dim3(256), 0, st, (const SegJob *)jobs_buf.p,
                     (const uint32_t *)ctx->jump_polys.p);
  HIPCHK(ctx, hipGetLastError());
  SYNCCHK(ctx, hipStreamSynchronize(st));
  return MH_OK;
}

int32_t mt_state_words(mh_ctx *ctx, hipStream_t st, const uint32_t *key624, int32_t pos, int64_t count, DevBuf &out,
                       DevBuf &key_buf) {
  if (pos < 0 || pos > 624) return arg_fail(ctx, MH_E_ARG, "MT19937 state position outside 0..624");
  MH_TRY(ensure(ctx, out, 4 * (size_t)count + 64));
  MH_TRY(ensure(ctx, key_buf, 4 * 624));
  HIPCHK(ctx, hipMemcpyAsync(key_buf.p, key624, 4 * 624, hipMemcpyHostToDevice, st));
  hipLaunchKernelGGL(k_mt_state, dim3(1), dim3(256), 0, st, (const uint32_t *)key_buf.p, pos, count,
                     (uint32_t *)out.p);
  HIPCHK(ctx, hipGetLastError());
  SYNCCHK(ctx, hipStreamSynchronize(st));
  return MH_OK;
}

namespace {

struct UnitPlan {
  NodeIdx ni;
  int64_t p_min, p_max, n, n_fo_words, n_shuf_words;
  uint32_t s_tloc, s_tlen, s_shuf, s_fo;
  int64_t w_tloc, w_tlen, w_fo, w_shuf;
  int64_t j_off;
  TplSet *out;
};

int32_t decode_parallel(mh_ctx *ctx, const std::vector<DecJob> &dec, int64_t *d_status, bool *done) {
  hipStream_t st = ctx->stream;
  *done = false;
  const int64_t div = 128;
  const int64_t minw = 64;
  std::vector<ChunkJob> cj;
  std::vector<int64_t> s0;
  std::vector<int32_t> first(dec.size() + 1, 0);
  for (size_t u = 0; u < dec.size(); u++) {
    first[u] = (int32_t)cj.size();
    double i = (double)(dec[u].n - 1);
    for (int64_t b = 0; b < dec[u].n_words;) {
      int64_t size = DC_CHUNK;
      while (size > minw && (double)size * (double)div > i) size >>= 1;
      cj.push_back(ChunkJob{dec[u].words, dec[u].n_words, b, dec[u].j, 0, (int32_t)size});
      s0.push_back(b == 0 ? dec[u].n - 1 : (i >= 1.0 ? (int64_t)llround(i) : 0));
      double rem = (double)size;
      while (rem > 0 && i >= 1.0) {
        uint32_t ii = (uint32_t)i, m = ii;
        m |= m >> 1; m |= m >> 2; m |= m >> 4; m |= m >> 8; m |= m >> 16;
        const double rate = (i + 1.0) / ((double)m + 1.0);
        const double lo = (double)((m >> 1) + 1);
        const double need = (i - lo + 1.0) / rate;
        if (need >= rem) { i -= rem * rate; rem = 0; }
        else { i = lo - 1.0; rem -= need; }
      }
      b += size;
    }
  }
  first[dec.size()] = (int32_t)cj.size();
  const int64_t C = (int64_t)cj.size();
  if (C == 0) {
    *done = true;
    return MH_OK;
  }
  const int32_t U = (int32_t)dec.size();
  const int64_t tail_at = (int64_t)1 << 15;
  std::vector<int32_t> tail_c(U, -1);
  for (int32_t u = 0; u < U; u++)
    for (int32_t c = first[u]; c < first[u + 1] && tail_at > 0; c++)
      if (s0[c] < tail_at) {
        tail_c[u] = c;
        for (int32_t k = c; k < first[u + 1]; k++) cj[k].tail = 1;
        break;
      }
  const int32_t tile_sz = DR_TILE;
  std::vector<DecTile> tiles;
  for (int32_t u = 0; u < U; u++) {
    const int32_t ft = (int32_t)tiles.size();
    for (int32_t b = first[u]; b < first[u + 1]; b += tile_sz)
      tiles.push_back(DecTile{u, b, std::min(b + tile_sz, first[u + 1]), ft});
  }
  const int32_t T = (int32_t)tiles.size();
  const size_t bytes = ((sizeof(ChunkJob) * C + 15) / 16) * 16 + 8 * C * 2 + 8 * U * 2 + sizeof(TailJob) * U +
                       sizeof(DecTile) * (T + 1) + 4 * C * 2 + 8 * C + 512;
  MH_TRY(ensure(ctx, ctx->dec_buf, bytes));
  char *p = (char *)ctx->dec_buf.p;
  ChunkJob *d_jobs = (ChunkJob *)p;
  int64_t *d_s0 = (int64_t *)(p + ((sizeof(ChunkJob) * C + 15) / 16) * 16);
  int64_t *d_s1 = d_s0 + C;
  int64_t *d_ndraw = d_s1 + C;
  int64_t *d_rem = d_ndraw + U;
  TailJob *d_tail = (TailJob *)(d_rem + U);
  DecTile *d_tiles = (DecTile *)(d_tail + U);
  int32_t *d_count = (int32_t *)(d_tiles + T + 1);
  int32_t *d_todo = d_count + C;
  int32_t *d_margin = d_todo + C;
  int32_t *d_ntodo = d_margin + 2 * C;
  std::vector<int64_t> ndraw(U);
  for (int32_t u = 0; u < U; u++) ndraw[u] = dec[u].n;
  std::vector<TailJob> tj;
  for (int32_t u = 0; u < U; u++)
    if (tail_c[u] >= 0 && dec[u].n > 0)
      tj.push_back(TailJob{dec[u].words, dec[u].n_words, cj[tail_c[u]].base, d_s1 + tail_c[u], dec[u].j, dec[u].status});
  HIPCHK(ctx, hipMemcpyAsync(d_jobs, cj.data(), sizeof(ChunkJob) * C, hipMemcpyHostToDevice, st));
  HIPCHK(ctx, hipMemcpyAsync(d_s0, s0.data(), 8 * C, hipMemcpyHostToDevice, st));
  HIPCHK(ctx, hipMemcpyAsync(d_tiles, tiles.data(), sizeof(DecTile) * T, hipMemcpyHostToDevice, st));
  HIPCHK(ctx, hipMemcpyAsync(d_ndraw, ndraw.data(), 8 * U, hipMemcpyHostToDevice, st));
  if (!tj.empty()) HIPCHK(ctx, hipMemcpyAsync(d_tail, tj.data(), sizeof(TailJob) * tj.size(), hipMemcpyHostToDevice, st));
  HIPCHK(ctx, hipMemsetAsync(d_ntodo, 0, 8, st));
  const unsigned grid = (unsigned)std::min<int64_t>(C, 4096);
  constexpr int MAX_PASSES = 64;
  const int PASS_BATCH = 24;
  hipLaunchKernelGGL(k_decode_chunks<false>, dim3(grid), dim3(DC_THREADS), 0, st, (const ChunkJob *)d_jobs,
                     (const int32_t *)nullptr, (const int32_t *)nullptr, (int32_t)C, (const int64_t *)d_s0, d_count,
                     d_margin);
  HIPCHK(ctx, hipGetLastError());
  bool conv = false;
  int passes = 1;
  while (passes < MAX_PASSES) {
    int32_t *cur = d_ntodo;
    for (int k = 0; k < PASS_BATCH; k++, passes++) {
      cur = d_ntodo + (passes & 1);
      int32_t *nxt = d_ntodo + ((passes + 1) & 1);
      const unsigned g = passes < 4 ? grid : std::min(grid, 1024u);
      hipLaunchKernelGGL(k_decode_resolve, dim3(T), dim3(DR_THREADS), 0, st, (const DecTile *)d_tiles,
                         (const int64_t *)d_ndraw, (const int32_t *)d_count, (const int32_t *)d_margin, d_s0, d_s1,
                         d_todo, cur, nxt, d_rem);
      hipLaunchKernelGGL(k_decode_chunks<false>, dim3(g), dim3(DC_THREADS), 0, st, (const ChunkJob *)d_jobs,
                         (const int32_t *)d_todo, (const int32_t *)cur, (int32_t)C, (const int64_t *)d_s0, d_count,
                         d_margin);
    }
    HIPCHK(ctx, hipGetLastError());
    int64_t *hs = pinned_small(ctx);
    if (!hs) return arg_fail(ctx, MH_E_OOM, "pinned host memory");
    HIPCHK(ctx, hipMemcpyAsync(hs + 32, cur, 4, hipMemcpyDeviceToHost, st));
    SYNCCHK(ctx, hipStreamSynchronize(st));
    const int32_t h_ntodo = (int32_t)(hs[32] & 0xffffffff);
    if (h_ntodo == 0) {
      conv = true;
      break;
    }
  }
  ctx->dec_passes = passes;
  if (!conv) return MH_OK;
  hipLaunchKernelGGL(k_decode_chunks<true>, dim3(grid), dim3(DC_THREADS), 0, st, (const ChunkJob *)d_jobs,
                     (const int32_t *)nullptr, (const int32_t *)nullptr, (int32_t)C, (const int64_t *)d_s1, d_count,
                     d_margin);
  HIPCHK(ctx, hipGetLastError());
  for (int32_t u = 0; u < U; u++)
    if (dec[u].n > 0 && tail_c[u] < 0) HIPCHK(ctx, hipMemcpyAsync(dec[u].status, d_rem + u, 8, hipMemcpyDeviceToDevice, st));
  if (!tj.empty()) {
    hipLaunchKernelGGL(k_decode_tail, dim3((unsigned)tj.size()), dim3(64), 0, st, (const TailJob *)d_tail);
    HIPCHK(ctx, hipGetLastError());
  }
  for (size_t u = 0; u < dec.size(); u++)
    if (dec[u].n > 0) HIPCHK(ctx, hipMemsetAsync(dec[u].j, 0, 4, st));
  SYNCCHK(ctx, hipStreamSynchronize(st));
  *done = true;
  return MH_OK;
}

template <class KIn>
static hipError_t perm_sort(void *tmp, size_t &tmp_bytes, KIn keys_in, uint32_t *keys_out, uint32_t *vals_out,
                            size_t n, unsigned end_bit, hipStream_t st) {
  return lsd_sort_pairs_iota(tmp, tmp_bytes, keys_in, keys_out, vals_out, (int64_t)n, end_bit, st);
}

struct BatchPerm {
  int64_t *ts, *tsh;
};

int32_t finish_unit(mh_ctx *ctx, UnitPlan &u, const uint32_t *words, const uint32_t *jarr, double p, int32_t rlen,
                    const double *d_cum, int32_t n_tlen, int32_t rng_mode, bool exact, int64_t *d_m,
                    uint32_t *d_flag, int lane = 0, int phase = 0, const BatchPerm *bp = nullptr) {
  hipStream_t st = lane == 0 ? ctx->stream : lane == 1 ? ctx->stream2 : ctx->xstream[lane - 2];
  ctx->stage_stream = lane ? st : nullptr;
  struct Restore {
    mh_ctx *c;
    ~Restore() { c->stage_stream = nullptr; }
  } restore{ctx};
  mh::DevBuf *S4 = lane == 0 ? ctx->s + 4 : lane == 1 ? ctx->lane2 : ctx->xlane[lane - 2];
  mh::DevBuf &perm_tmp = lane == 0 ? ctx->perm_tmp : S4[7];
  void *scan_partials = lane == 0 ? ctx->scan_partials.p : lane == 1 ? ctx->scan_partials2.p : ctx->xscan[lane - 2].p;
  const int64_t n = u.n;
  const uint32_t *w_tloc = words + u.w_tloc, *w_tlen = words + u.w_tlen, *w_fo = words + u.w_fo;
  int64_t *ts = bp ? bp->ts + u.j_off : (int64_t *)S4[0].p;
  int64_t *ts_shuf = (int64_t *)S4[1].p, *te = (int64_t *)S4[2].p;
  uint32_t *sk = (uint32_t *)S4[4].p, *sv = (uint32_t *)S4[5].p;
  int32_t *nxt = (int32_t *)S4[6].p;
  const bool permute = rng_mode == MH_RNG_MITTY && n > 1 && !bp;
  uint8_t *keep = (uint8_t *)S4[3].p;
  int64_t *flag_idx = (int64_t *)ctx->s[11].p;
  int64_t *tot = (int64_t *)((char *)ctx->d_small.p + 128 + 64 * lane);
  const double log_q = std::log(1.0 - p);
  GeoFlags fl{flag_idx, d_flag, 1024};

  if (phase != 2) {
    stage_begin(ctx, "sample_geometric_scan");
    if (!exact) {
      HIPCHK(ctx, device_scan_sum<int64_t>(st, n, LoadGeo{w_tloc, p, log_q, fl}, StoreTs{ts, u.p_min + 1, u.ni},
                                           scan_partials, tot));
    } else {
      int64_t *g = (int64_t *)ctx->s[12].p;
      uint32_t nflag = 0;
      HIPCHK(ctx, hipMemsetAsync(d_flag, 0, 4, st));
      hipLaunchKernelGGL(k_geo_array, dim3(grid_for(n, 256, INT32_MAX)), dim3(256), 0, st, n, w_tloc, p, log_q, fl, g);
      HIPCHK(ctx, hipMemcpyAsync(&nflag, d_flag, 4, hipMemcpyDeviceToHost, st));
      SYNCCHK(ctx, hipStreamSynchronize(st));
      auto host_geo = [&](const uint32_t *ww) {
        double U = (((int32_t)(ww[0] >> 5)) * 67108864.0 + ((int32_t)(ww[1] >> 6))) / 9007199254740992.0;
        return (int64_t)std::ceil(std::log1p(-U) / std::log(1.0 - p));
      };
      if (ctx->force_geo && p < 0.333333333333333333333333) {
        std::vector<uint32_t> hw(2 * (size_t)n);
        std::vector<int64_t> hg((size_t)n);
        HIPCHK(ctx, hipMemcpy(hw.data(), w_tloc, 8 * (size_t)n, hipMemcpyDeviceToHost));
        for (int64_t k = 0; k < n; k++) hg[k] = host_geo(hw.data() + 2 * k);
        HIPCHK(ctx, hipMemcpy(g, hg.data(), 8 * (size_t)n, hipMemcpyHostToDevice));
      } else {
        if (nflag > 1024) return arg_fail(ctx, MH_E_ARG, "too many near-integer geometric quotients");
        std::vector<int64_t> idx(nflag);
        if (nflag) HIPCHK(ctx, hipMemcpy(idx.data(), flag_idx, 8 * nflag, hipMemcpyDeviceToHost));
        for (int64_t k : idx) {
          uint32_t ww[2];
          HIPCHK(ctx, hipMemcpy(ww, w_tloc + 2 * k, 8, hipMemcpyDeviceToHost));
          int64_t gv = host_geo(ww);
          HIPCHK(ctx, hipMemcpy(g + k, &gv, 8, hipMemcpyHostToDevice));
        }
      }
      HIPCHK(ctx, hipMemsetAsync(d_flag, 0, 4, st));
      HIPCHK(ctx, device_scan<int64_t>(st, n, LoadArr{g}, StoreTs{ts, u.p_min + 1, u.ni}, OpSum{}, (int64_t)0,
                                       (int64_t *)scan_partials, tot));
    }
    stage_end(ctx);

    if (permute) {
      stage_begin(ctx, "sample_permutation");
      unsigned end_bit = 1;
      while (end_bit < 32 && ((int64_t)1 << end_bit) < n) end_bit++;
      size_t tmp = 0;
      HIPCHK(ctx, perm_sort(nullptr, tmp, jarr, sk, sv, (size_t)n, end_bit, st));
      MH_TRY(ensure(ctx, perm_tmp, tmp + 256));
      HIPCHK(ctx, perm_sort(perm_tmp.p, tmp, jarr, sk, sv, (size_t)n, end_bit, st));
      HIPCHK(ctx, hipMemsetAsync(nxt, 0xff, 4 * (size_t)n, st));
      hipLaunchKernelGGL(k_perm_heads, dim3(grid_for(n, 256, INT32_MAX)), dim3(256), 0, st, n, (const uint32_t *)sk,
                         (const uint32_t *)sv, nxt);
      HIPCHK(ctx, hipGetLastError());
      stage_end(ctx);
    }
  }
  if (phase == 1) return MH_OK;

  const int64_t *ts_use = bp && rng_mode == MH_RNG_MITTY && n > 1 ? bp->tsh + u.j_off : ts;
  if (permute) {
    stage_begin(ctx, "sample_permutation");
    hipLaunchKernelGGL(k_perm_chase, dim3(grid_for(n, 256, INT32_MAX)), dim3(256), 0, st, (int64_t)0, n,
                       (const uint32_t *)sk, (const uint32_t *)sv, (const int32_t *)nxt, (const int64_t *)ts, ts_shuf);
    HIPCHK(ctx, hipGetLastError());
    stage_end(ctx);
    ts_use = ts_shuf;
  }

  stage_begin(ctx, "sample_tlen_compact");
  hipLaunchKernelGGL(k_tlen, dim3(grid_for((n + TLEN_PER - 1) / TLEN_PER, 256, INT32_MAX)), dim3(256), 8 * n_tlen, st,
                     n, w_tlen, d_cum, n_tlen,
                     (int64_t)rlen, u.p_max, ts_use, te, keep);
  HIPCHK(ctx, hipGetLastError());
  HIPCHK(ctx, device_scan_sum<int64_t>(st, n, LoadKeep{keep},
                                       StoreCompact{keep, ts_use, te, (int64_t *)u.out->pos0.p,
                                                    (int64_t *)u.out->pos1.p, (int64_t)rlen, w_fo,
                                                    (int8_t *)u.out->fo0.p,
                                                    u.out->has_n0 ? (int32_t *)u.out->n0.p : nullptr},
                                       scan_partials, d_m));
  stage_end(ctx);
  return MH_OK;
}

}

struct SampleState {
  std::vector<UnitPlan> plan;
  int32_t n_units = 0, rng_mode = 0, rlen = 0, n_tlen = 0, n_lanes = 1;
  bool two_lanes = false, batch = false;
  double p = 0;
  int64_t j_total = 0, nn = 0;
  uint32_t *words = nullptr, *jall = nullptr;
  double *d_cum = nullptr;
  int64_t *d_m = nullptr, *d_status = nullptr;
  uint32_t *d_flags = nullptr;
  BatchPerm bp{nullptr, nullptr};
  std::vector<hipEvent_t> ev;
  int32_t n_pending = 0;
  ~SampleState() {
    for (hipEvent_t e : ev)
      if (e) (void)hipEventDestroy(e);
  }
};

static void plan_unit_words(UnitPlan &q, int64_t p_min, int64_t p_max, uint64_t seed, double p, int32_t rng_mode,
                            int64_t &words_total) {
  q.p_min = p_min;
  q.p_max = p_max;
  q.n = (int64_t)((double)(q.p_max - q.p_min) * p * 1.2);
  if (q.n < 0) q.n = 0;
  HostMT sr;
  sr.seed((uint32_t)seed);
  q.s_tloc = (uint32_t)sr.interval(0xfffffffeull);
  q.s_tlen = (uint32_t)sr.interval(0xfffffffeull);
  q.s_shuf = (uint32_t)sr.interval(0xfffffffeull);
  q.s_fo = (uint32_t)sr.interval(0xfffffffeull);
  q.n_fo_words = (q.n + 3) / 4 + 1;
  q.n_shuf_words = rng_mode == MH_RNG_MITTY ? shuffle_words_alloc(q.n) : 0;
  auto take = [&](int64_t cnt) {
    int64_t at = words_total;
    words_total = (words_total + cnt + 4 + 3) & ~(int64_t)3;
    return at;
  };
  q.w_tloc = take(2 * q.n);
  q.w_tlen = take(2 * q.n);
  q.w_fo = take(q.n_fo_words);
  q.w_shuf = take(q.n_shuf_words);
}

static void unit_seg_jobs(uint32_t *words, const UnitPlan &q, std::vector<SegJob> &jobs, int64_t &kmax) {
  const int64_t SEG_WORDS = seg_words();
  auto add_stream = [&](uint32_t *out, int64_t count, uint32_t seed) {
    for (int64_t k = 0; k * SEG_WORDS < count; k++) {
      int64_t s0 = k * SEG_WORDS;
      jobs.push_back(SegJob{out, s0, std::min(SEG_WORDS, count - s0), seed, (int32_t)k});
      kmax = std::max(kmax, k);
    }
  };
  add_stream(words + q.w_tloc, 2 * q.n, q.s_tloc);
  add_stream(words + q.w_tlen, 2 * q.n, q.s_tlen);
  add_stream(words + q.w_fo, q.n_fo_words, q.s_fo);
  add_stream(words + q.w_shuf, q.n_shuf_words, q.s_shuf);
}

static int32_t sample_head(mh_ctx *ctx, SampleState &S, int32_t n_units, const int32_t *tpl_ids, const int64_t *p_min,
                           const int64_t *p_max, const uint64_t *seeds, double p, int32_t rlen, const double *cum_tlen,
                           int32_t n_tlen, int32_t rng_mode, const NodeIdx *nidx) {
  for (int32_t u = 0; u < n_units; u++)
    if (seeds[u] > 0xffffffffull)
      return arg_fail(ctx, MH_E_SEED, "Seed value " + std::to_string(seeds[u]) + " is out of range 0 - 4294967295");
  if (n_tlen <= 0 || n_tlen > 8192) return arg_fail(ctx, MH_E_ARG, "cum_tlen must have 1..8192 entries");
  if (rng_mode != MH_RNG_MITTY && rng_mode != MH_RNG_PHILOX) return arg_fail(ctx, MH_E_ARG, "unknown rng_mode");
  MH_TRY(tpl_resolve_all(ctx));
  hipStream_t st = ctx->stream;

  std::vector<UnitPlan> plan(n_units);
  int64_t words_total = 0, j_total = 0, n_max = 1;
  for (int32_t u = 0; u < n_units; u++) {
    UnitPlan &q = plan[u];
    plan_unit_words(q, p_min[u], p_max[u], seeds[u], p, rng_mode, words_total);
    if (q.n > ((int64_t)1 << 30) - 8) return arg_fail(ctx, MH_E_ARG, "region too large for one work unit");
    q.j_off = j_total; j_total += q.n + 4;
    n_max = std::max(n_max, q.n);
    TplSet &ts = ctx->tsets[tpl_ids[u]];
    MH_TRY(wait_unused(ctx, ts.used, ts.used_set));
    MH_TRY(ensure(ctx, ts.fo0, q.n + 16));
    MH_TRY(ensure(ctx, ts.pos0, 8 * (q.n + 16)));
    MH_TRY(ensure(ctx, ts.pos1, 8 * (q.n + 16)));
    q.ni = nidx ? nidx[u] : NodeIdx{};
    ts.n_draws = q.n;
    ts.has_n0 = q.ni.nd != nullptr;
    if (ts.has_n0) MH_TRY(ensure(ctx, ts.n0, 4 * (q.n + 16)));
    ts.valid = false;
    q.out = &ts;
  }
  const int64_t nn = n_max + 1;
  ctx->batch_left = 0;
  for (const UnitPlan &q : plan) ctx->batch_left += q.n;
  PrefetchedWords &pw = ctx->pf_words;
  const bool have_words = rng_mode == MH_RNG_MITTY && pw.valid && pw.p == p && pw.seeds.size() == (size_t)n_units &&
                          std::equal(pw.seeds.begin(), pw.seeds.end(), seeds) &&
                          std::equal(pw.p_min.begin(), pw.p_min.end(), p_min) &&
                          std::equal(pw.p_max.begin(), pw.p_max.end(), p_max) && pw.words_total == words_total;
  pw.valid = false;
  if (have_words) std::swap(ctx->s[0], pw.buf);
  MH_TRY(ensure(ctx, ctx->s[0], 4 * (size_t)words_total + 64));
  MH_TRY(ensure(ctx, ctx->s[3], 4 * (size_t)j_total + 64));
  MH_TRY(ensure(ctx, ctx->s[4], 8 * nn));
  MH_TRY(ensure(ctx, ctx->s[5], 8 * nn));
  MH_TRY(ensure(ctx, ctx->s[6], 8 * nn));
  MH_TRY(ensure(ctx, ctx->s[7], nn));
  MH_TRY(ensure(ctx, ctx->s[8], 4 * (nn + 1)));
  MH_TRY(ensure(ctx, ctx->s[9], 4 * (nn + 1)));
  MH_TRY(ensure(ctx, ctx->s[10], 4 * nn));
  MH_TRY(ensure(ctx, ctx->s[11], 8 * 1024));
  int n_lanes = std::max(1, std::min(2, (int)n_units));
  const bool two_lanes = n_lanes > 1;
  for (int l = 2; l < n_lanes; l++)
    if (!ctx->xstream[l - 2]) {
      int lo = 0, hi = 0;
      (void)hipDeviceGetStreamPriorityRange(&lo, &hi);
      HIPCHK(ctx, hipStreamCreateWithPriority(&ctx->xstream[l - 2], hipStreamNonBlocking, hi));
      HIPCHK(ctx, hipEventCreateWithFlags(&ctx->ev_xjoin[l - 2], hipEventDisableTiming));
    }
  for (int l = 1; l < n_lanes; l++) {
    mh::DevBuf *L = l == 1 ? ctx->lane2 : ctx->xlane[l - 2];
    MH_TRY(ensure(ctx, L[0], 8 * nn));
    MH_TRY(ensure(ctx, L[1], 8 * nn));
    MH_TRY(ensure(ctx, L[2], 8 * nn));
    MH_TRY(ensure(ctx, L[3], nn));
    MH_TRY(ensure(ctx, L[4], 4 * (nn + 1)));
    MH_TRY(ensure(ctx, L[5], 4 * (nn + 1)));
    MH_TRY(ensure(ctx, L[6], 4 * nn));
    MH_TRY(ensure(ctx, l == 1 ? ctx->scan_partials2 : ctx->xscan[l - 2],
                  std::max<size_t>(16 * scan_partials_count(nn + 1) + 64, scan_lb_scratch_bytes<int64_t>(nn + 1))));
  }
  MH_TRY(ensure(ctx, ctx->s[13], 8 * (size_t)n_tlen + 64));
  MH_TRY(ensure(ctx, ctx->s[1], 64 * (size_t)n_units + 64));
  MH_TRY(ensure(ctx, ctx->d_small, 8192 + 256));
  MH_TRY(ensure(ctx, ctx->scan_partials, std::max<size_t>(16 * scan_partials_count(nn + 1) + 64,
                                                           scan_lb_scratch_bytes<int64_t>(nn + 1))));
  uint32_t *words = (uint32_t *)ctx->s[0].p, *jall = (uint32_t *)ctx->s[3].p;
  double *d_cum = (double *)ctx->s[13].p;
  int64_t *d_m = (int64_t *)ctx->s[1].p;
  int64_t *d_status = d_m + n_units;
  uint32_t *d_flags = (uint32_t *)(d_status + n_units);
  HIPCHK(ctx, hipMemsetAsync(ctx->s[1].p, 0, 64 * (size_t)n_units + 64, st));
  HIPCHK(ctx, hipMemcpyAsync(d_cum, cum_tlen, 8 * n_tlen, hipMemcpyHostToDevice, st));

  stage_begin(ctx, "sample");
  if (rng_mode == MH_RNG_MITTY) {
    std::vector<SegJob> jobs;
    std::vector<DecJob> dec;
    int64_t kmax = 0;
    const int64_t SEG_WORDS = seg_words();
    for (int32_t u = 0; u < n_units; u++) {
      UnitPlan &q = plan[u];
      if (q.n == 0) continue;
      unit_seg_jobs(words, q, jobs, kmax);
      dec.push_back(DecJob{words + q.w_shuf, q.n_shuf_words, q.n, jall + q.j_off, d_status + u});
    }
    if (!jobs.empty()) {
      MH_TRY(ensure_polys(ctx, st, kmax, SEG_WORDS));
      MH_TRY(ensure(ctx, ctx->s[2], sizeof(SegJob) * jobs.size() + sizeof(DecJob) * dec.size() + 64));
      SegJob *d_jobs = (SegJob *)ctx->s[2].p;
      DecJob *d_dec = (DecJob *)((char *)ctx->s[2].p + ((sizeof(SegJob) * jobs.size() + 15) / 16) * 16);
      HIPCHK(ctx, hipMemcpyAsync(d_jobs, jobs.data(), sizeof(SegJob) * jobs.size(), hipMemcpyHostToDevice, st));
      HIPCHK(ctx, hipMemcpyAsync(d_dec, dec.data(), sizeof(DecJob) * dec.size(), hipMemcpyHostToDevice, st));
      if (!have_words) {
        stage_begin(ctx, "sample_mt_segments");
        hipLaunchKernelGGL(k_mt_segments, dim3((unsigned)jobs.size()), dim3(256), 0, st, (const SegJob *)d_jobs,
                           (const uint32_t *)ctx->jump_polys.p);
        HIPCHK(ctx, hipGetLastError());
        stage_end(ctx);
      }
      stage_begin(ctx, "sample_shuffle_decode");
      bool done = false;
      if (!ctx->decode_sequential) MH_TRY(decode_parallel(ctx, dec, d_status, &done));
      if (!done) {
        hipLaunchKernelGGL(k_shuffle_decode2, dim3((unsigned)dec.size()), dim3(DC_THREADS), 0, st,
                           (const DecJob *)d_dec);
        HIPCHK(ctx, hipGetLastError());
      }
      stage_end(ctx);
      SYNCCHK(ctx, hipStreamSynchronize(st));
    }
  } else {
    for (int32_t u = 0; u < n_units; u++) {
      UnitPlan &q = plan[u];
      if (q.n == 0) continue;
      uint64_t key = ((uint64_t)q.s_tloc << 32) | q.s_tlen;
      hipLaunchKernelGGL(k_philox_words, dim3(grid_for((2 * q.n + 3) / 4, 256, INT32_MAX)), dim3(256), 0, st,
                         words + q.w_tloc, 2 * q.n, key, 1u);
      hipLaunchKernelGGL(k_philox_words, dim3(grid_for((2 * q.n + 3) / 4, 256, INT32_MAX)), dim3(256), 0, st,
                         words + q.w_tlen, 2 * q.n, key, 2u);
      hipLaunchKernelGGL(k_philox_words, dim3(grid_for((q.n_fo_words + 3) / 4, 256, INT32_MAX)), dim3(256), 0, st,
                         words + q.w_fo, q.n_fo_words, key, 3u);
      HIPCHK(ctx, hipGetLastError());
    }
  }

  if (two_lanes) {
    HIPCHK(ctx, hipEventRecord(ctx->ev_fork, st));
    HIPCHK(ctx, hipStreamWaitEvent(ctx->stream2, ctx->ev_fork, 0));
    for (int l = 2; l < n_lanes; l++) HIPCHK(ctx, hipStreamWaitEvent(ctx->xstream[l - 2], ctx->ev_fork, 0));
  }
  const bool batch = rng_mode == MH_RNG_MITTY && j_total < ((int64_t)1 << 30) && n_units <= PK_UNITS;
  if (batch) {
    MH_TRY(ensure(ctx, ctx->pb[0], 8 * (size_t)j_total + 64));
    MH_TRY(ensure(ctx, ctx->pb[1], 8 * (size_t)j_total + 64));
    for (int b = 2; b < 6; b++) MH_TRY(ensure(ctx, ctx->pb[b], 4 * (size_t)j_total + 64));
    BatchPerm bp{(int64_t *)ctx->pb[0].p, (int64_t *)ctx->pb[1].p};
    for (int32_t u = 0, k = 0; u < n_units; u++) {
      if (plan[u].n == 0) continue;
      MH_TRY(finish_unit(ctx, plan[u], words, jall + plan[u].j_off, p, rlen, d_cum, n_tlen, rng_mode, false, d_m + u,
                         d_flags + u, k++ % n_lanes, 1, &bp));
    }
    if (two_lanes) {
      HIPCHK(ctx, hipEventRecord(ctx->ev_join, ctx->stream2));
      HIPCHK(ctx, hipStreamWaitEvent(st, ctx->ev_join, 0));
      for (int l = 2; l < n_lanes; l++) {
        HIPCHK(ctx, hipEventRecord(ctx->ev_xjoin[l - 2], ctx->xstream[l - 2]));
        HIPCHK(ctx, hipStreamWaitEvent(st, ctx->ev_xjoin[l - 2], 0));
      }
    }
    stage_begin(ctx, "sample_permutation");
    std::vector<int64_t> uo(n_units), un(n_units);
    for (int32_t u = 0; u < n_units; u++) {
      uo[u] = plan[u].j_off;
      un[u] = plan[u].n;
    }
    int64_t *d_uo = (int64_t *)ctx->s[12].p;
    MH_TRY(ensure(ctx, ctx->s[12], 16 * (size_t)n_units + 64));
    d_uo = (int64_t *)ctx->s[12].p;
    HIPCHK(ctx, hipMemcpyAsync(d_uo, uo.data(), 8 * n_units, hipMemcpyHostToDevice, st));
    HIPCHK(ctx, hipMemcpyAsync(d_uo + n_units, un.data(), 8 * n_units, hipMemcpyHostToDevice, st));
    uint32_t *gk = (uint32_t *)ctx->pb[2].p, *sk = (uint32_t *)ctx->pb[3].p, *sv = (uint32_t *)ctx->pb[4].p;
    int32_t *nxt = (int32_t *)ctx->pb[5].p;
    hipLaunchKernelGGL(k_perm_keys, dim3(grid_for(j_total, 256, INT32_MAX)), dim3(256), 0, st, j_total,
                       (const uint32_t *)jall, (const int64_t *)d_uo, (const int64_t *)(d_uo + n_units), n_units, gk,
                       nxt);
    HIPCHK(ctx, hipGetLastError());
    unsigned end_bit = 1;
    while (end_bit < 32 && ((int64_t)1 << end_bit) < j_total) end_bit++;
    size_t tmp = 0;
    HIPCHK(ctx, perm_sort(nullptr, tmp, gk, sk, sv, (size_t)j_total, end_bit, st));
    MH_TRY(ensure(ctx, ctx->pb_tmp, tmp + 256));
    HIPCHK(ctx, perm_sort(ctx->pb_tmp.p, tmp, gk, sk, sv, (size_t)j_total, end_bit, st));
    hipLaunchKernelGGL(k_perm_heads, dim3(grid_for(j_total, 256, INT32_MAX)), dim3(256), 0, st, j_total,
                       (const uint32_t *)sk, (const uint32_t *)sv, nxt);
    HIPCHK(ctx, hipGetLastError());
    stage_end(ctx);
    S.bp = bp;
  } else {
    for (int32_t u = 0, k = 0; u < n_units; u++) {
      if (plan[u].n == 0) continue;
      MH_TRY(finish_unit(ctx, plan[u], words, jall + plan[u].j_off, p, rlen, d_cum, n_tlen, rng_mode, false, d_m + u,
                         d_flags + u, k++ % n_lanes));
    }
  }
  S.plan = std::move(plan);
  S.n_units = n_units;
  S.rng_mode = rng_mode;
  S.rlen = rlen;
  S.n_tlen = n_tlen;
  S.n_lanes = n_lanes;
  S.two_lanes = two_lanes;
  S.batch = batch;
  S.p = p;
  S.j_total = j_total;
  S.nn = nn;
  S.words = words;
  S.jall = jall;
  S.d_cum = d_cum;
  S.d_m = d_m;
  S.d_status = d_status;
  S.d_flags = d_flags;
  return MH_OK;
}

static int32_t sample_tail(mh_ctx *ctx, SampleState &S, int64_t *out_n) {
  hipStream_t st = ctx->stream;
  std::vector<UnitPlan> &plan = S.plan;
  const int32_t n_units = S.n_units, rng_mode = S.rng_mode, rlen = S.rlen, n_tlen = S.n_tlen, n_lanes = S.n_lanes;
  const bool two_lanes = S.two_lanes;
  const double p = S.p;
  const int64_t j_total = S.j_total, nn = S.nn;
  uint32_t *words = S.words, *jall = S.jall;
  double *d_cum = S.d_cum;
  int64_t *d_m = S.d_m, *d_status = S.d_status;
  uint32_t *d_flags = S.d_flags;
  if (S.batch) {
    const BatchPerm &bp = S.bp;
    const uint32_t *sk = (const uint32_t *)ctx->pb[3].p, *sv = (const uint32_t *)ctx->pb[4].p;
    const int32_t *nxt = (const int32_t *)ctx->pb[5].p;
    stage_begin(ctx, "sample_permutation");
    hipLaunchKernelGGL(k_perm_chase, dim3(grid_for(j_total, 256, INT32_MAX)), dim3(256), 0, st, (int64_t)0, j_total,
                       sk, sv, nxt, (const int64_t *)bp.ts, bp.tsh);
    HIPCHK(ctx, hipGetLastError());
    stage_end(ctx);
    if (two_lanes) {
      HIPCHK(ctx, hipEventRecord(ctx->ev_fork, st));
      HIPCHK(ctx, hipStreamWaitEvent(ctx->stream2, ctx->ev_fork, 0));
      for (int l = 2; l < n_lanes; l++) HIPCHK(ctx, hipStreamWaitEvent(ctx->xstream[l - 2], ctx->ev_fork, 0));
    }
    for (int32_t u = 0, k = 0; u < n_units; u++) {
      if (plan[u].n == 0) continue;
      MH_TRY(finish_unit(ctx, plan[u], words, jall + plan[u].j_off, p, rlen, d_cum, n_tlen, rng_mode, false, d_m + u,
                         d_flags + u, k++ % n_lanes, 2, &bp));
    }
  }
  if (two_lanes) {
    HIPCHK(ctx, hipEventRecord(ctx->ev_join, ctx->stream2));
    HIPCHK(ctx, hipStreamWaitEvent(st, ctx->ev_join, 0));
    for (int l = 2; l < n_lanes; l++) {
      HIPCHK(ctx, hipEventRecord(ctx->ev_xjoin[l - 2], ctx->xstream[l - 2]));
      HIPCHK(ctx, hipStreamWaitEvent(st, ctx->ev_xjoin[l - 2], 0));
    }
  }
  std::vector<int64_t> hm(n_units), hstat(n_units);
  std::vector<uint32_t> hflag(n_units);
  int64_t *hs = pinned_small(ctx);
  const size_t rb_bytes = 20 * (size_t)n_units;
  if (hs && rb_bytes <= 3072) {
    HIPCHK(ctx, hipMemcpyAsync(hs + 64, d_m, rb_bytes, hipMemcpyDeviceToHost, st));
    SYNCCHK(ctx, hipStreamSynchronize(st));
    std::memcpy(hm.data(), hs + 64, 8 * n_units);
    std::memcpy(hstat.data(), hs + 64 + n_units, 8 * n_units);
    std::memcpy(hflag.data(), hs + 64 + 2 * n_units, 4 * n_units);
  } else {
    HIPCHK(ctx, hipMemcpyAsync(hm.data(), d_m, 8 * n_units, hipMemcpyDeviceToHost, st));
    HIPCHK(ctx, hipMemcpyAsync(hstat.data(), d_status, 8 * n_units, hipMemcpyDeviceToHost, st));
    HIPCHK(ctx, hipMemcpyAsync(hflag.data(), d_flags, 4 * n_units, hipMemcpyDeviceToHost, st));
    SYNCCHK(ctx, hipStreamSynchronize(st));
  }

  for (int32_t u = 0; u < n_units; u++) {
    UnitPlan &q = plan[u];
    if (q.n == 0) continue;
    if (ctx->force_fixup) hstat[u] = 1;
    if (ctx->force_geo) hflag[u] = 1;
    if (hstat[u] == 0 && hflag[u] == 0) continue;
    if (rng_mode == MH_RNG_MITTY && hstat[u] != 0) {
      hipLaunchKernelGGL(k_shuffle_decode, dim3(1), dim3(SD_THREADS), 0, st, q.s_shuf, q.n, jall + q.j_off);
      HIPCHK(ctx, hipGetLastError());
    }
    MH_TRY(ensure(ctx, ctx->s[12], 8 * (size_t)nn));
    HIPCHK(ctx, hipMemsetAsync(d_flags + u, 0, 4, st));
    MH_TRY(finish_unit(ctx, q, words, jall + q.j_off, p, rlen, d_cum, n_tlen, rng_mode, hflag[u] != 0, d_m + u,
                       d_flags + u));
    HIPCHK(ctx, hipMemcpyAsync(&hm[u], d_m + u, 8, hipMemcpyDeviceToHost, st));
    SYNCCHK(ctx, hipStreamSynchronize(st));
    ctx->fixups++;
  }
  stage_end(ctx);
  for (int32_t u = 0; u < n_units; u++) {
    TplSet &ts = *plan[u].out;
    ts.n = plan[u].n == 0 ? 0 : hm[u];
    ts.rlen = rlen;
    ts.valid = true;
    if (out_n) out_n[u] = ts.n;
  }
  return MH_OK;
}

__global__ void k_unit_result(const int64_t *m, const int64_t *status, const uint32_t *flag, int64_t *out) {
  if (threadIdx.x == 0) {
    out[0] = *m;
    out[1] = *status;
    out[2] = (int64_t)*flag;
  }
}

static int32_t sample_tail_async(mh_ctx *ctx, const std::shared_ptr<SampleState> &Sp) {
  SampleState &S = *Sp;
  std::vector<UnitPlan> &plan = S.plan;
  const int32_t n_units = S.n_units;
  hipStream_t st = ctx->stream, l1 = ctx->stream2;
  const BatchPerm &bp = S.bp;
  const uint32_t *sk = (const uint32_t *)ctx->pb[3].p, *sv = (const uint32_t *)ctx->pb[4].p;
  const int32_t *nxt = (const int32_t *)ctx->pb[5].p;
  HIPCHK(ctx, hipEventRecord(ctx->ev_fork, st));
  HIPCHK(ctx, hipStreamWaitEvent(l1, ctx->ev_fork, 0));
  S.ev.assign(n_units, nullptr);
  for (int32_t u = 0; u < n_units; u++) {
    UnitPlan &q = plan[u];
    TplSet &ts = *q.out;
    if (q.n == 0) {
      ts.n = 0;
      ts.rlen = S.rlen;
      ts.valid = true;
      continue;
    }
    ctx->stage_stream = l1;
    stage_begin(ctx, "sample_permutation");
    const int64_t k0 = q.j_off, k1 = q.j_off + q.n + 4;
    hipLaunchKernelGGL(k_perm_chase, dim3(grid_for(k1 - k0, 256, INT32_MAX)), dim3(256), 0, l1, k0, k1, sk, sv, nxt,
                       (const int64_t *)bp.ts, bp.tsh);
    stage_end(ctx);
    ctx->stage_stream = nullptr;
    HIPCHK(ctx, hipGetLastError());
    MH_TRY(finish_unit(ctx, q, S.words, S.jall + q.j_off, S.p, S.rlen, S.d_cum, S.n_tlen, S.rng_mode, false,
                       S.d_m + u, S.d_flags + u, 1, 2, &bp));
    hipLaunchKernelGGL(k_unit_result, dim3(1), dim3(64), 0, l1, (const int64_t *)(S.d_m + u),
                       (const int64_t *)(S.d_status + u), (const uint32_t *)(S.d_flags + u), ctx->d_units + 4 * u);
    HIPCHK(ctx, hipGetLastError());
    HIPCHK(ctx, hipEventCreateWithFlags(&S.ev[u], hipEventDisableTiming));
    HIPCHK(ctx, hipEventRecord(S.ev[u], l1));
    ts.pend = u;
    S.n_pending++;
  }
  stage_end(ctx);
  if (S.n_pending) ctx->tail_state = Sp;
  return MH_OK;
}

int32_t tpl_resolve(mh_ctx *ctx, TplSet &ts) {
  if (ts.pend < 0) return MH_OK;
  const int32_t u = ts.pend;
  ts.pend = -1;
  auto Sp = std::static_pointer_cast<SampleState>(ctx->tail_state);
  if (!Sp || u >= Sp->n_units || Sp->plan[u].out != &ts)
    return arg_fail(ctx, MH_E_STATE, "template set of a lost sampling batch");
  SampleState &S = *Sp;
  UnitPlan &q = S.plan[u];
  hipStream_t st = ctx->stream;
  SYNCCHK(ctx, hipEventSynchronize(S.ev[u]));
  const volatile int64_t *r = ctx->h_units + 4 * u;
  int64_t m = r[0];
  const int64_t status = ctx->force_fixup ? 1 : r[1];
  const uint32_t flag = ctx->force_geo ? 1u : (uint32_t)r[2];
  HIPCHK(ctx, hipStreamWaitEvent(st, S.ev[u], 0));
  if (status != 0 || flag != 0) {
    if (S.rng_mode == MH_RNG_MITTY && status != 0) {
      hipLaunchKernelGGL(k_shuffle_decode, dim3(1), dim3(SD_THREADS), 0, st, q.s_shuf, q.n, S.jall + q.j_off);
      HIPCHK(ctx, hipGetLastError());
    }
    MH_TRY(ensure(ctx, ctx->s[12], 8 * (size_t)S.nn));
    HIPCHK(ctx, hipMemsetAsync(S.d_flags + u, 0, 4, st));
    MH_TRY(finish_unit(ctx, q, S.words, S.jall + q.j_off, S.p, S.rlen, S.d_cum, S.n_tlen, S.rng_mode, flag != 0,
                       S.d_m + u, S.d_flags + u));
    HIPCHK(ctx, hipMemcpyAsync(&m, S.d_m + u, 8, hipMemcpyDeviceToHost, st));
    SYNCCHK(ctx, hipStreamSynchronize(st));
    ctx->fixups++;
  }
  ts.n = m;
  ts.rlen = S.rlen;
  ts.valid = true;
  if (--S.n_pending == 0) ctx->tail_state.reset();
  return MH_OK;
}

int32_t tpl_resolve_all(mh_ctx *ctx) {
  auto Sp = std::static_pointer_cast<SampleState>(ctx->tail_state);
  if (!Sp) return MH_OK;
  for (UnitPlan &q : Sp->plan)
    if (q.out && q.out->pend >= 0) MH_TRY(tpl_resolve(ctx, *q.out));
  return MH_OK;
}

int32_t prefetch_words(mh_ctx *ctx, hipStream_t st, int32_t n_units, const int64_t *p_min, const int64_t *p_max,
                       const uint64_t *seeds, double p) {
  PrefetchedWords &pw = ctx->pf_words;
  pw.valid = false;
  std::vector<UnitPlan> plan(n_units);
  int64_t words_total = 0;
  for (int32_t u = 0; u < n_units; u++) {
    plan_unit_words(plan[u], p_min[u], p_max[u], seeds[u], p, MH_RNG_MITTY, words_total);
    if (plan[u].n > ((int64_t)1 << 30) - 8) return MH_OK;
  }
  MH_TRY(ensure(ctx, pw.buf, 4 * (size_t)words_total + 64));
  std::vector<SegJob> jobs;
  int64_t kmax = 0;
  for (const UnitPlan &q : plan)
    if (q.n > 0) unit_seg_jobs((uint32_t *)pw.buf.p, q, jobs, kmax);
  if (jobs.empty() || ctx->jump_k < kmax + 1 || ctx->jump_seg != seg_words()) return MH_OK;
  MH_TRY(ensure(ctx, pw.jobs, sizeof(SegJob) * jobs.size() + 64));
  HIPCHK(ctx, hipMemcpyAsync(pw.jobs.p, jobs.data(), sizeof(SegJob) * jobs.size(), hipMemcpyHostToDevice, st));
  hipLaunchKernelGGL(k_mt_segments, dim3((unsigned)jobs.size()), dim3(256), 0, st, (const SegJob *)pw.jobs.p,
                     (const uint32_t *)ctx->jump_polys.p);
  HIPCHK(ctx, hipGetLastError());
  SYNCCHK(ctx, hipStreamSynchronize(st));
  pw.p = p;
  pw.seeds.assign(seeds, seeds + n_units);
  pw.p_min.assign(p_min, p_min + n_units);
  pw.p_max.assign(p_max, p_max + n_units);
  pw.words_total = words_total;
  pw.valid = true;
  return MH_OK;
}

int32_t sample_units_async(mh_ctx *ctx, int32_t n_units, const int32_t *tpl_ids, const int64_t *p_min,
                           const int64_t *p_max, const uint64_t *seeds, double p, int32_t rlen, const double *cum_tlen,
                           int32_t n_tlen, int32_t rng_mode, const NodeIdx *nidx) {
  if (!ctx->h_units) {
    if (hipHostMalloc((void **)&ctx->h_units, 32 * (size_t)PK_UNITS, hipHostMallocMapped | hipHostMallocCoherent) !=
        hipSuccess) {
      ctx->h_units = nullptr;
      return arg_fail(ctx, MH_E_OOM, "pinned host memory");
    }
    void *d = nullptr;
    HIPCHK(ctx, hipHostGetDevicePointer(&d, ctx->h_units, 0));
    ctx->d_units = (int64_t *)d;
  }
  auto S = std::make_shared<SampleState>();
  MH_TRY(sample_head(ctx, *S, n_units, tpl_ids, p_min, p_max, seeds, p, rlen, cum_tlen, n_tlen, rng_mode, nidx));
  if (!S->batch || !S->two_lanes) return sample_tail(ctx, *S, nullptr);
  return sample_tail_async(ctx, S);
}

int32_t sample_units(mh_ctx *ctx, int32_t n_units, const int32_t *tpl_ids, const int64_t *p_min, const int64_t *p_max,
                     const uint64_t *seeds, double p, int32_t rlen, const double *cum_tlen, int32_t n_tlen,
                     int32_t rng_mode, int64_t *out_n, const NodeIdx *nidx) {
  SampleState S;
// ... 6 lines not shown
```

Measured before the change: 1.713 billion.

## Make parallel shuffle decode sync-free with device-side convergence and fallback

Replaces the host-polled convergence loop in the parallel shuffle decode with a fixed batch of resolve/chunk passes that exit early on the device through a convergence flag. The sequential block decode fallback is now always launched but returns immediately unless the pass count did not converge. The stream synchronizations after decoding are removed, so sampling can overlap later work without a host round-trip. It also adds a separate fault slot for the prefetch thread, host tables kept alive for the async copies, and stats counters. The trade-off is that a fixed number of mostly empty kernels always launch, and fallback now depends on the device flag.

After: 1.718 billion, median of 2. No clear change (+0.3%).

```diff
diff --git a/include/mitty_hip.h b/include/mitty_hip.h
--- a/include/mitty_hip.h
+++ b/include/mitty_hip.h
@@ -217,8 +217,10 @@
 #define MH_DEC_SEQUENTIAL 1
 #define MH_DEC_FORCE_FIXUP 2
 #define MH_DEC_FORCE_GEO 4
+#define MH_DEC_FORCE_BLOCKSEQ 8
 int32_t mh_set_decode_mode(mh_ctx *ctx, int32_t mode);
 int32_t mh_fixup_count(mh_ctx *ctx, int64_t *n);
+int32_t mh_sample_stats(mh_ctx *ctx, int64_t out[4]);
 
 #ifdef __cplusplus
 }
diff --git a/mitty_amd/_native.py b/mitty_amd/_native.py
--- a/mitty_amd/_native.py
+++ b/mitty_amd/_native.py
@@ -17,7 +17,7 @@
            'mh_release_haplotype', 'mh_expand_variant', 'mh_sample_templates', 'mh_sample_templates_span', 'mh_set_templates',
            'mh_get_templates', 'mh_templates_export', 'mh_templates_import', 'mh_emit_reads', 'mh_emit_prepare', 'mh_emit_reads_async', 'mh_emit_collect', 'mh_output_size', 'mh_output_fetch', 'mh_output_reset', 'mh_host_alloc', 'mh_host_free', 'mh_device_cache_trim', 'mh_device_live_bytes',
            'mh_read_batch', 'mh_set_corruption', 'mh_set_corruption_stream', 'mh_get_corruption_stream', 'mh_stage_times', 'mh_enable_timing', 'mh_sample_units', 'mh_sample_units_async', 'mh_templates_count',
-           'mh_use_templates', 'mh_release_templates', 'mh_mt_window_at', 'mh_fixup_count', 'mh_set_emit_mode', 'mh_set_decode_mode',
+           'mh_use_templates', 'mh_release_templates', 'mh_mt_window_at', 'mh_fixup_count', 'mh_sample_stats', 'mh_set_emit_mode', 'mh_set_decode_mode',
            'mh_emit_reads_range', 'mh_emit_measure', 'mh_count_kept', 'mh_bam_set_refs', 'mh_bam_add_fastq', 'mh_bam_add_output',
            'mh_bam_records', 'mh_bam_set_capacity', 'mh_bam_set_spill_dir', 'mh_bam_spilled', 'mh_bam_export', 'mh_bam_import', 'mh_bam_sort', 'mh_bam_write', 'mh_bam_write_gpu', 'mh_bam_reset', 'mh_bam_partition', 'mh_bam_partition_fetch', 'mh_bam_import_tie', 'mh_bam_sorted_head', 'mh_bam_write_part', 'mh_bam_bai_runs', 'mh_corrupt_fastq', 'mh_bgzf_compress', 'mh_bgzf_eof', 'mh_bgzf_compress_device', 'mh_bgzf_compress_gpu', 'mh_output_bgzf',
            'mh_output_bgzf_range', 'mh_output_bgzf_pair', 'mh_output_bgzf_wait', 'mh_output_fetch_async',
@@ -175,6 +175,7 @@
   _sig(L, 'mh_release_templates', [c_vp, c_i32])
   _sig(L, 'mh_mt_window_at', [ctypes.c_uint32, c_u64, c_vp])
   _sig(L, 'mh_fixup_count', [c_vp, P_i64])
+  _sig(L, 'mh_sample_stats', [c_vp, P_i64])
   _sig(L, 'mh_set_emit_mode', [c_vp, c_i32])
   _sig(L, 'mh_set_decode_mode', [c_vp, c_i32])
   _lib = L
@@ -610,6 +611,11 @@
     self._chk(self._L.mh_fixup_count(self._h, ctypes.byref(n)))
     return n.value
 
+  def sample_stats(self):
+    out = (c_i64 * 4)()
+    self._chk(self._L.mh_sample_stats(self._h, out))
+    return dict(zip(('adopted', 'built', 'fallbacks', 'fixups'), (int(v) for v in out)))
+
   def set_templates(self, fo0, pos0, pos1, rlen):
     fo0 = np.ascontiguousarray(fo0, dtype=np.int8)
     pos0 = np.ascontiguousarray(pos0, dtype=np.int64)
diff --git a/mitty_amd/csrc/mh_api.hip b/mitty_amd/csrc/mh_api.hip
--- a/mitty_amd/csrc/mh_api.hip
+++ b/mitty_amd/csrc/mh_api.hip
@@ -48,15 +48,22 @@
   return code;
 }
 
+static thread_local int tl_check_slot = -1;
+static int check_slot(const mh_ctx *ctx) { return tl_check_slot >= 0 ? tl_check_slot : (ctx ? ctx->fault_slot : 0); }
+
 bool scan_fault_pending(const mh_ctx *ctx) {
   const uint32_t *h = scan_fault_host();
-  return h && __atomic_load_n(h + (ctx ? ctx->fault_slot : 0), __ATOMIC_ACQUIRE) != 0;
-}
-
-void lane_thread_enter(mh_ctx *ctx) { scan_fault_slot = ctx->fault_slot; }
+  return h && __atomic_load_n(h + check_slot(ctx), __ATOMIC_ACQUIRE) != 0;
+}
+
+void lane_thread_enter(mh_ctx *ctx, int slot) {
+  (void)ctx;
+  scan_fault_slot = slot;
+  tl_check_slot = slot;
+}
 
 int32_t scan_fault_fail(mh_ctx *ctx) {
-  const uint32_t v = scan_fault_take(ctx ? ctx->fault_slot : 0);
+  const uint32_t v = scan_fault_take(check_slot(ctx));
   if (v & 2u) return arg_fail(ctx, MH_E_STATE, "single-pass writer: a qname part exceeded the splice's bound (internal)");
   if (v & 4u) return arg_fail(ctx, MH_E_STATE, "single-pass writer: the arena reservation was too small (internal)");
   return arg_fail(ctx, MH_E_STATE, "a look-back scan's wait timed out (a broken ticket base or scratch): its offsets "
@@ -434,7 +441,9 @@
   {
     static std::atomic<int> next{0};
     ctx->fault_slot = 1 + next++ % (SCAN_FAULT_SLOTS - 1);
+    ctx->pf_fault_slot = 1 + next++ % (SCAN_FAULT_SLOTS - 1);
     (void)scan_fault_take(ctx->fault_slot);
+    (void)scan_fault_take(ctx->pf_fault_slot);
   }
   int prio_lo = 0, prio_hi = 0;
   (void)hipSetDevice(device);
@@ -621,7 +630,7 @@
   };
   int32_t rc_lane = MH_OK;
   std::thread t1([&]() {
-    lane_thread_enter(ctx);
+    lane_thread_enter(ctx, ctx->fault_slot);
     if (hipSetDevice(ctx->device) != hipSuccess) {
       rc_lane = MH_E_HIP;
       return;
@@ -801,7 +810,7 @@
       const VarSet &v1 = ctx->vsets[vsets[i0 + 1]];
       int32_t rc1 = MH_OK;
       std::thread t1([&]() {
-        lane_thread_enter(ctx);
+        lane_thread_enter(ctx, ctx->fault_slot);
         try {
           const hipError_t e = hipSetDevice(ctx->device);
           if (e != hipSuccess) {
@@ -887,7 +896,7 @@
   ctx->pf_rc = MH_OK;
   ctx->pf_thread = std::thread([ctx, jobs, uh, useeds, p]() {
     int32_t rc = MH_OK;
-    lane_thread_enter(ctx);
+    lane_thread_enter(ctx, ctx->pf_fault_slot);
     try {
       const hipError_t e = hipSetDevice(ctx->device);
       if (e != hipSuccess) rc = hip_fail(ctx, e, "hipSetDevice (prefetch)", __FILE__, __LINE__);
@@ -1588,16 +1597,27 @@
 }
 
 int32_t mh_set_decode_mode(mh_ctx *ctx, int32_t mode) {
-  if (!ctx || mode < 0 || mode > (MH_DEC_SEQUENTIAL | MH_DEC_FORCE_FIXUP | MH_DEC_FORCE_GEO)) return MH_E_ARG;
+  if (!ctx || mode < 0 || mode > (MH_DEC_SEQUENTIAL | MH_DEC_FORCE_FIXUP | MH_DEC_FORCE_GEO | MH_DEC_FORCE_BLOCKSEQ))
+    return MH_E_ARG;
   ctx->decode_sequential = (mode & MH_DEC_SEQUENTIAL) != 0;
   ctx->force_fixup = (mode & MH_DEC_FORCE_FIXUP) != 0;
   ctx->force_geo = (mode & MH_DEC_FORCE_GEO) != 0;
+  ctx->force_blockseq = (mode & MH_DEC_FORCE_BLOCKSEQ) != 0;
   return MH_OK;
 }
 
 int32_t mh_fixup_count(mh_ctx *ctx, int64_t *n) {
   if (!ctx || !n) return MH_E_ARG;
   *n = ctx->fixups;
+  return MH_OK;
+}
+
+int32_t mh_sample_stats(mh_ctx *ctx, int64_t out[4]) {
+  if (!ctx || !out) return MH_E_ARG;
+  out[0] = ctx->heads_adopted;
+  out[1] = ctx->heads_built;
+  out[2] = ctx->dec_fallbacks;
+  out[3] = ctx->fixups;
   return MH_OK;
 }
 
diff --git a/mitty_amd/csrc/mh_internal.h b/mitty_amd/csrc/mh_internal.h
--- a/mitty_amd/csrc/mh_internal.h
+++ b/mitty_amd/csrc/mh_internal.h
@@ -224,6 +224,7 @@
 
 struct mh_ctx {
   int fault_slot = 0;
+  int pf_fault_slot = 0;
   int device = 0;
   hipStream_t stream = nullptr;
   hipStream_t stream2 = nullptr;
@@ -250,6 +251,7 @@
   mh::DevBuf jump_polys;
   int64_t jump_k = 0, jump_seg = 0;
   int64_t fixups = 0;
+  int64_t heads_adopted = 0, heads_built = 0, dec_fallbacks = 0;
   std::map<int32_t, mh::VarSet> vsets;
   std::vector<mh::Hap> hap_spare;
   mh::DevBuf perm_tmp;
@@ -305,6 +307,7 @@
   bool decode_sequential = false;
   bool force_fixup = false;
   bool force_geo = false;
+  bool force_blockseq = false;
 
   mh::DevBuf out1, out2;
   int64_t used1 = 0, used2 = 0;
@@ -352,6 +355,7 @@
   } while (0)
 
 int32_t scan_fault_fail(mh_ctx *ctx);
+void lane_thread_enter(mh_ctx *ctx, int slot);
 #define SYNCCHK(ctx, call)                                                    \
   do {                                                                        \
     HIPCHK(ctx, call);                                                        \
diff --git a/mitty_amd/csrc/mh_sample.hip b/mitty_amd/csrc/mh_sample.hip
--- a/mitty_amd/csrc/mh_sample.hip
+++ b/mitty_amd/csrc/mh_sample.hip
@@ -181,9 +181,14 @@
 constexpr int DC_PER = 4;
 constexpr int DC_CHUNK = DC_THREADS * DC_PER;
 
-__global__ void __launch_bounds__(DC_THREADS) k_shuffle_decode2(const DecJob *jobs) {
+__global__ void __launch_bounds__(DC_THREADS) k_shuffle_decode2(const DecJob *jobs, const int32_t *pred, int32_t force,
+                                                                uint32_t *fb) {
   __shared__ int32_t wsum[DC_WAVES];
   __shared__ int32_t s_tot;
+  if (pred) {
+    if (*pred == 0 && !force) return;
+    if (blockIdx.x == 0 && threadIdx.x == 0) *fb = 1u;
+  }
   const DecJob job = jobs[blockIdx.x];
   const int t = threadIdx.x, lane = t & 63, wave = t >> 6;
   if (t == 0 && job.n > 0) job.j[0] = 0;
@@ -414,11 +419,12 @@
 __global__ void __launch_bounds__(DC_THREADS) k_decode_chunks(const ChunkJob *jobs, const int32_t *todo,
                                                               const int32_t *n_todo, int32_t n_all,
                                                               const int64_t *start, int32_t *count,
-                                                              int32_t *margin) {
+                                                              int32_t *margin, int32_t *conv, int32_t pass) {
   __shared__ int32_t wsum[DC_WAVES];
   __shared__ int32_t wlo[DC_WAVES], whi[DC_WAVES];
   __shared__ int32_t s_tot;
   const int32_t n = todo ? *n_todo : n_all;
+  if (conv && n == 0 && blockIdx.x == 0 && threadIdx.x == 0 && *conv == 0) *conv = pass;
   for (int32_t i = blockIdx.x; i < n; i += gridDim.x) {
     decode_chunk<WRITE>(jobs, todo ? todo[i] : i, start, count, margin, wsum, wlo, whi, s_tot);
     __syncthreads();
@@ -445,9 +451,11 @@
 __global__ void __launch_bounds__(DR_THREADS) k_decode_resolve(const DecTile *tiles, const int64_t *n_draws,
                                                                const int32_t *count, const int32_t *margin,
                                                                int64_t *s0, int64_t *s1, int32_t *todo,
-                                                               int32_t *n_todo, int32_t *n_next, int64_t *rem) {
+                                                               int32_t *n_todo, int32_t *n_next, int64_t *rem,
+                                                               const int32_t *conv) {
   __shared__ int64_t wsum[DR_THREADS / 64];
   const int t = threadIdx.x, lane = t & 63, wave = t >> 6;
+  if (*conv != 0) return;
   const DecTile tl = tiles[blockIdx.x];
   if (blockIdx.x == 0 && t == 0) *n_next = 0;
   int64_t before = 0;
@@ -955,13 +963,25 @@
   TplSet *out;
 };
 
-int32_t decode_parallel(mh_ctx *ctx, const std::vector<DecJob> &dec, int64_t *d_status, bool *done) {
+struct HeadTables {
+  std::vector<SegJob> jobs;
+  std::vector<DecJob> dec;
+  std::vector<ChunkJob> cj;
+  std::vector<int64_t> s0, ndraw, uo, un;
+  std::vector<DecTile> tiles;
+  std::vector<TailJob> tj;
+  std::vector<double> cum;
+};
+
+int32_t decode_parallel(mh_ctx *ctx, HeadTables &HT, const DecJob *d_dec, uint32_t *d_fb) {
   hipStream_t st = ctx->stream;
-  *done = false;
+  const std::vector<DecJob> &dec = HT.dec;
+  std::vector<ChunkJob> &cj = HT.cj;
+  std::vector<int64_t> &s0 = HT.s0, &ndraw = HT.ndraw;
+  std::vector<DecTile> &tiles = HT.tiles;
+  std::vector<TailJob> &tj = HT.tj;
   const int64_t div = 128;
   const int64_t minw = 64;
-  std::vector<ChunkJob> cj;
-  std::vector<int64_t> s0;
   std::vector<int32_t> first(dec.size() + 1, 0);
   for (size_t u = 0; u < dec.size(); u++) {
     first[u] = (int32_t)cj.size();
@@ -986,10 +1006,8 @@
   }
   first[dec.size()] = (int32_t)cj.size();
   const int64_t C = (int64_t)cj.size();
-  if (C == 0) {
-    *done = true;
-    return MH_OK;
-  }
+  ctx->dec_passes = 0;
+  if (C == 0) return MH_OK;
   const int32_t U = (int32_t)dec.size();
   const int64_t tail_at = (int64_t)1 << 15;
   std::vector<int32_t> tail_c(U, -1);
@@ -1001,7 +1019,6 @@
         break;
       }
   const int32_t tile_sz = DR_TILE;
-  std::vector<DecTile> tiles;
   for (int32_t u = 0; u < U; u++) {
     const int32_t ft = (int32_t)tiles.size();
     for (int32_t b = first[u]; b < first[u + 1]; b += tile_sz)
@@ -1023,9 +1040,8 @@
   int32_t *d_todo = d_count + C;
   int32_t *d_margin = d_todo + C;
   int32_t *d_ntodo = d_margin + 2 * C;
-  std::vector<int64_t> ndraw(U);
+  ndraw.resize(U);
   for (int32_t u = 0; u < U; u++) ndraw[u] = dec[u].n;
-  std::vector<TailJob> tj;
   for (int32_t u = 0; u < U; u++)
     if (tail_c[u] >= 0 && dec[u].n > 0)
       tj.push_back(TailJob{dec[u].words, dec[u].n_words, cj[tail_c[u]].base, d_s1 + tail_c[u], dec[u].j, dec[u].status});
@@ -1034,45 +1050,32 @@
   HIPCHK(ctx, hipMemcpyAsync(d_tiles, tiles.data(), sizeof(DecTile) * T, hipMemcpyHostToDevice, st));
   HIPCHK(ctx, hipMemcpyAsync(d_ndraw, ndraw.data(), 8 * U, hipMemcpyHostToDevice, st));
   if (!tj.empty()) HIPCHK(ctx, hipMemcpyAsync(d_tail, tj.data(), sizeof(TailJob) * tj.size(), hipMemcpyHostToDevice, st));
-  HIPCHK(ctx, hipMemsetAsync(d_ntodo, 0, 8, st));
+  int32_t *d_conv = d_ntodo + 2;
+  HIPCHK(ctx, hipMemsetAsync(d_ntodo, 0, 16, st));
   const unsigned grid = (unsigned)std::min<int64_t>(C, 4096);
-  constexpr int MAX_PASSES = 64;
-  const int PASS_BATCH = 24;
+  const int PASS_BATCH = 32;
   hipLaunchKernelGGL(k_decode_chunks<false>, dim3(grid), dim3(DC_THREADS), 0, st, (const ChunkJob *)d_jobs,
                      (const int32_t *)nullptr, (const int32_t *)nullptr, (int32_t)C, (const int64_t *)d_s0, d_count,
-                     d_margin);
+                     d_margin, (int32_t *)nullptr, 0);
   HIPCHK(ctx, hipGetLastError());
-  bool conv = false;
   int passes = 1;
-  while (passes < MAX_PASSES) {
-    int32_t *cur = d_ntodo;
-    for (int k = 0; k < PASS_BATCH; k++, passes++) {
-      cur = d_ntodo + (passes & 1);
-      int32_t *nxt = d_ntodo + ((passes + 1) & 1);
-      const unsigned g = passes < 4 ? grid : std::min(grid, 1024u);
-      hipLaunchKernelGGL(k_decode_resolve, dim3(T), dim3(DR_THREADS), 0, st, (const DecTile *)d_tiles,
-                         (const int64_t *)d_ndraw, (const int32_t *)d_count, (const int32_t *)d_margin, d_s0, d_s1,
-                         d_todo, cur, nxt, d_rem);
-      hipLaunchKernelGGL(k_decode_chunks<false>, dim3(g), dim3(DC_THREADS), 0, st, (const ChunkJob *)d_jobs,
-                         (const int32_t *)d_todo, (const int32_t *)cur, (int32_t)C, (const int64_t *)d_s0, d_count,
-                         d_margin);
-    }
-    HIPCHK(ctx, hipGetLastError());
-    int64_t *hs = pinned_small(ctx);
-    if (!hs) return arg_fail(ctx, MH_E_OOM, "pinned host memory");
-    HIPCHK(ctx, hipMemcpyAsync(hs + 32, cur, 4, hipMemcpyDeviceToHost, st));
-    SYNCCHK(ctx, hipStreamSynchronize(st));
-    const int32_t h_ntodo = (int32_t)(hs[32] & 0xffffffff);
-    if (h_ntodo == 0) {
-      conv = true;
-      break;
-    }
-  }
+  int32_t *cur = d_ntodo;
+  for (int k = 0; k < PASS_BATCH; k++, passes++) {
+    cur = d_ntodo + (passes & 1);
+    int32_t *nxt = d_ntodo + ((passes + 1) & 1);
+    const unsigned g = passes < 4 ? grid : std::min(grid, 1024u);
+    hipLaunchKernelGGL(k_decode_resolve, dim3(T), dim3(DR_THREADS), 0, st, (const DecTile *)d_tiles,
+                       (const int64_t *)d_ndraw, (const int32_t *)d_count, (const int32_t *)d_margin, d_s0, d_s1,
+                       d_todo, cur, nxt, d_rem, (const int32_t *)d_conv);
+    hipLaunchKernelGGL(k_decode_chunks<false>, dim3(g), dim3(DC_THREADS), 0, st, (const ChunkJob *)d_jobs,
+                       (const int32_t *)d_todo, (const int32_t *)cur, (int32_t)C, (const int64_t *)d_s0, d_count,
+                       d_margin, d_conv, (int32_t)passes);
+  }
+  HIPCHK(ctx, hipGetLastError());
   ctx->dec_passes = passes;
-  if (!conv) return MH_OK;
   hipLaunchKernelGGL(k_decode_chunks<true>, dim3(grid), dim3(DC_THREADS), 0, st, (const ChunkJob *)d_jobs,
                      (const int32_t *)nullptr, (const int32_t *)nullptr, (int32_t)C, (const int64_t *)d_s1, d_count,
-                     d_margin);
+                     d_margin, (int32_t *)nullptr, 0);
   HIPCHK(ctx, hipGetLastError());
   for (int32_t u = 0; u < U; u++)
     if (dec[u].n > 0 && tail_c[u] < 0) HIPCHK(ctx, hipMemcpyAsync(dec[u].status, d_rem + u, 8, hipMemcpyDeviceToDevice, st));
@@ -1082,8 +1085,9 @@
   }
   for (size_t u = 0; u < dec.size(); u++)
     if (dec[u].n > 0) HIPCHK(ctx, hipMemsetAsync(dec[u].j, 0, 4, st));
-  SYNCCHK(ctx, hipStreamSynchronize(st));
-  *done = true;
+  hipLaunchKernelGGL(k_shuffle_decode2, dim3((unsigned)dec.size()), dim3(DC_THREADS), 0, st, d_dec,
+                     (const int32_t *)cur, (int32_t)(ctx->force_blockseq ? 1 : 0), d_fb);
+  HIPCHK(ctx, hipGetLastError());
   return MH_OK;
 }
 
@@ -1216,9 +1220,15 @@
   int64_t *d_m = nullptr, *d_status = nullptr;
   uint32_t *d_flags = nullptr;
   BatchPerm bp{nullptr, nullptr};
+  uint32_t *d_fb = nullptr;
+  bool fb_counted = false;
+  HeadTables tables;
+  hipStream_t head_stream = nullptr;
+  bool head_read = false;
   std::vector<hipEvent_t> ev;
   int32_t n_pending = 0;
   ~SampleState() {
+    if (head_stream && !head_read) (void)hipStreamSynchronize(head_stream);
     for (hipEvent_t e : ev)
       if (e) (void)hipEventDestroy(e);
   }
@@ -1346,13 +1356,18 @@
   int64_t *d_m = (int64_t *)ctx->s[1].p;
   int64_t *d_status = d_m + n_units;
   uint32_t *d_flags = (uint32_t *)(d_status + n_units);
+  uint32_t *d_fb = d_flags + n_units;
+  HeadTables &T = S.tables;
+  S.head_stream = st;
+  ctx->heads_built++;
   HIPCHK(ctx, hipMemsetAsync(ctx->s[1].p, 0, 64 * (size_t)n_units + 64, st));
-  HIPCHK(ctx, hipMemcpyAsync(d_cum, cum_tlen, 8 * n_tlen, hipMemcpyHostToDevice, st));
+  T.cum.assign(cum_tlen, cum_tlen + n_tlen);
+  HIPCHK(ctx, hipMemcpyAsync(d_cum, T.cum.data(), 8 * n_tlen, hipMemcpyHostToDevice, st));
 
   stage_begin(ctx, "sample");
   if (rng_mode == MH_RNG_MITTY) {
-    std::vector<SegJob> jobs;
-    std::vector<DecJob> dec;
+    std::vector<SegJob> &jobs = T.jobs;
+    std::vector<DecJob> &dec = T.dec;
     int64_t kmax = 0;
     const int64_t SEG_WORDS = seg_words();
     for (int32_t u = 0; u < n_units; u++) {
@@ -1376,15 +1391,14 @@
         stage_end(ctx);
       }
       stage_begin(ctx, "sample_shuffle_decode");
-      bool done = false;
-      if (!ctx->decode_sequential) MH_TRY(decode_parallel(ctx, dec, d_status, &done));
-      if (!done) {
+      if (!ctx->decode_sequential) {
+        MH_TRY(decode_parallel(ctx, T, (const DecJob *)d_dec, d_fb));
+      } else {
         hipLaunchKernelGGL(k_shuffle_decode2, dim3((unsigned)dec.size()), dim3(DC_THREADS), 0, st,
-                           (const DecJob *)d_dec);
+                           (const DecJob *)d_dec, (const int32_t *)nullptr, 0, d_fb);
         HIPCHK(ctx, hipGetLastError());
       }
       stage_end(ctx);
-      SYNCCHK(ctx, hipStreamSynchronize(st));
     }
   } else {
     for (int32_t u = 0; u < n_units; u++) {
@@ -1426,7 +1440,9 @@
       }
     }
     stage_begin(ctx, "sample_permutation");
-    std::vector<int64_t> uo(n_units), un(n_units);
+    std::vector<int64_t> &uo = T.uo, &un = T.un;
+    uo.resize(n_units);
+    un.resize(n_units);
     for (int32_t u = 0; u < n_units; u++) {
       uo[u] = plan[u].j_off;
       un[u] = plan[u].n;
@@ -1477,6 +1493,7 @@
   S.d_m = d_m;
   S.d_status = d_status;
   S.d_flags = d_flags;
+  S.d_fb = d_fb;
   return MH_OK;
 }
 
@@ -1522,18 +1539,26 @@
   std::vector<int64_t> hm(n_units), hstat(n_units);
   std::vector<uint32_t> hflag(n_units);
   int64_t *hs = pinned_small(ctx);
-  const size_t rb_bytes = 20 * (size_t)n_units;
+  const size_t rb_bytes = 20 * (size_t)n_units + 4;
+  uint32_t hfb = 0;
   if (hs && rb_bytes <= 3072) {
     HIPCHK(ctx, hipMemcpyAsync(hs + 64, d_m, rb_bytes, hipMemcpyDeviceToHost, st));
     SYNCCHK(ctx, hipStreamSynchronize(st));
     std::memcpy(hm.data(), hs + 64, 8 * n_units);
     std::memcpy(hstat.data(), hs + 64 + n_units, 8 * n_units);
     std::memcpy(hflag.data(), hs + 64 + 2 * n_units, 4 * n_units);
+    std::memcpy(&hfb, (const char *)(hs + 64) + 20 * (size_t)n_units, 4);
   } else {
     HIPCHK(ctx, hipMemcpyAsync(hm.data(), d_m, 8 * n_units, hipMemcpyDeviceToHost, st));
     HIPCHK(ctx, hipMemcpyAsync(hstat.data(), d_status, 8 * n_units, hipMemcpyDeviceToHost, st));
     HIPCHK(ctx, hipMemcpyAsync(hflag.data(), d_flags, 4 * n_units, hipMemcpyDeviceToHost, st));
+    HIPCHK(ctx, hipMemcpyAsync(&hfb, S.d_fb, 4, hipMemcpyDeviceToHost, st));
     SYNCCHK(ctx, hipStreamSynchronize(st));
+  }
+  S.head_read = true;
+  if (hfb != 0 && !S.fb_counted) {
+    S.fb_counted = true;
+    ctx->dec_fallbacks++;
   }
 
   for (int32_t u = 0; u < n_units; u++) {
@@ -1565,11 +1590,13 @@
   return MH_OK;
 }
 
-__global__ void k_unit_result(const int64_t *m, const int64_t *status, const uint32_t *flag, int64_t *out) {
+__global__ void k_unit_result(const int64_t *m, const int64_t *status, const uint32_t *flag, const uint32_t *fb,
+                              int64_t *out) {
   if (threadIdx.x == 0) {
     out[0] = *m;
     out[1] = *status;
     out[2] = (int64_t)*flag;
+    out[3] = (int64_t)*fb;
   }
 }
 
@@ -1604,7 +1631,8 @@
     MH_TRY(finish_unit(ctx, q, S.words, S.jall + q.j_off, S.p, S.rlen, S.d_cum, S.n_tlen, S.rng_mode, false,
                        S.d_m + u, S.d_flags + u, 1, 2, &bp));
     hipLaunchKernelGGL(k_unit_result, dim3(1), dim3(64), 0, l1, (const int64_t *)(S.d_m + u),
-                       (const int64_t *)(S.d_status + u), (const uint32_t *)(S.d_flags + u), ctx->d_units + 4 * u);
+                       (const int64_t *)(S.d_status + u), (const uint32_t *)(S.d_flags + u), (const uint32_t *)S.d_fb,
+                       ctx->d_units + 4 * u);
     HIPCHK(ctx, hipGetLastError());
     HIPCHK(ctx, hipEventCreateWithFlags(&S.ev[u], hipEventDisableTiming));
     HIPCHK(ctx, hipEventRecord(S.ev[u], l1));
@@ -1631,6 +1659,11 @@
   int64_t m = r[0];
   const int64_t status = ctx->force_fixup ? 1 : r[1];
   const uint32_t flag = ctx->force_geo ? 1u : (uint32_t)r[2];
+  S.head_read = true;
+  if (r[3] != 0 && !S.fb_counted) {
+    S.fb_counted = true;
+    ctx->dec_fallbacks++;
+  }
   HIPCHK(ctx, hipStreamWaitEvent(st, S.ev[u], 0));
   if (status != 0 || flag != 0) {
     if (S.rng_mode == MH_RNG_MITTY && status != 0) {
```
